# automl/TransformersCanDoBayesianInference

Hardware: AMD Instinct MI355X
Metric: synthetic datasets/sec (GP prior, bptt=2000) (higher is better)
Workload: dtype fp16; 1 GPU; priors.fast_gp, bptt=2000, num_features=18, emsize=512, nhead=4, nhid=1024, nlayers=6, 1000 bars (BASELINE.json configs[1]); per_gpu_batch=64, global_batch=64, aggregate_k_gradients=1, aggregate_streams=0, aggregate_stacked=False, seq_len=2000, parallelism=dp1, micro_batch_streams=2, eval_pos=weighted sampler(2000)

## Files before the change

include/pfn_hip.h:

```cpp
#ifndef PFN_HIP_H
#define PFN_HIP_H

#include <stddef.h>
#include <stdint.h>

#ifdef __cplusplus
extern "C" {
#endif

#define PFN_ABI_VERSION 10

enum {
  PFN_OK = 0,
  PFN_ERR_UNSUPPORTED = -1,
  PFN_ERR_ALIGNMENT = -2,
  PFN_ERR_LAUNCH = -3,
  PFN_ERR_ARGUMENT = -4,
};

enum { PFN_PREC_BF16 = 0,
       PFN_PREC_F32 = 1,
       PFN_PREC_FP16 = 2   };

typedef struct pfn_model_desc {
  int32_t num_features;
  int32_t emsize;
  int32_t nhead;
  int32_t nhid;
  int32_t nlayers;
  int32_t n_out;
  int32_t precision;
  float ln_eps;
  float dropout;
  int32_t schedule;
} pfn_model_desc;
enum { PFN_SCHED_TOP_LAYER_ALL_ROWS = 1,
       PFN_SCHED_FUSE_LN_WIDE = 2,
       PFN_SCHED_SEPARATE_LNBWD = 4,
       PFN_SCHED_NO_KEY_CENTERING = 16,
       PFN_SCHED_KEY_CENTERING = 64,
       PFN_SCHED_F32_RESIDUAL = 128,
       PFN_SCHED_FUSE_Q_PROJECTION = 32,
       PFN_SCHED_DETERMINISTIC = 8        };
int pfn_default_schedule(void);

int pfn_abi_version(void);
const char* pfn_last_error_string(void);
enum { PFN_TUNE_GEMM_NT_KERNEL = 0,
       PFN_TUNE_GEMM_TN_WRAP = 1,
       PFN_TUNE_FUSE_LNBWD = 2,
       PFN_TUNE_ATTN_PINGPONG = 4,
       PFN_TUNE_FUSE_LN_WIDE = 5,
       PFN_TUNE_GP_PLANES = 8,
       PFN_TUNE_FUSE_DELTA = 9,
       PFN_TUNE_GEMM_LN_ROWS = 7,
       PFN_TUNE_ATTN_BWD_GROUP = 10,
       PFN_TUNE_WGRAD_SPLITS = 11,
       PFN_TUNE_WGRAD_WAVES = 14,
       PFN_TUNE_LOSS_SCALE_TARGET = 15,
       PFN_TUNE_RESIDUAL16 = 16,
       PFN_TUNE_FUSE_Q_PROJECTION = 12,
       PFN_TUNE_KEY_CENTERING = 13,
       PFN_TUNE_ATTN_CACHE_SPLITS = 17,
       PFN_TUNE_TOP_LAYER_TEST_ROWS = 6  };
int pfn_set_tuning(int key, int value);
enum { PFN_PROF_ATTN_FWD = 0, PFN_PROF_ATTN_BWD_DELTA = 2, PFN_PROF_ATTN_BWD_KV = 4, PFN_PROF_ATTN_BWD_DQ = 6, PFN_PROF_GEMM_QKV = 8,
       PFN_PROF_GEMM_OUT_LN = 10, PFN_PROF_GEMM_LIN1 = 12, PFN_PROF_GEMM_LIN2_LN = 14, PFN_PROF_GEMM_DHPRE = 16, PFN_PROF_GEMM_DY1 = 18,
       PFN_PROF_GEMM_DCTX = 20, PFN_PROF_GEMM_DX = 22, PFN_PROF_WGRAD = 24, PFN_PROF_SLOTS = 26 };
int pfn_profile_enable(int on);
int pfn_profile_read(int slot, double* total_ms, int64_t* launches);

int pfn_param_layout(const pfn_model_desc* d, int64_t* offsets, int64_t* numels, int max_tensors);
int64_t pfn_param_count(const pfn_model_desc* d);
int64_t pfn_shadow_bytes(const pfn_model_desc* d);
int pfn_prepare_params(const pfn_model_desc* d, const float* params, void* shadow, void* stream);

int64_t pfn_workspace_bytes(const pfn_model_desc* d, int B, int S);
int64_t pfn_top_layer_rows(const pfn_model_desc* d, int B, int S, int sep, int use_dropout);
int pfn_stack_forward(const pfn_model_desc* d, const float* params, const void* shadow,
                      const float* x, int64_t x_st, int64_t x_sb,
                      const float* y, int64_t y_st, int64_t y_sb,
                      const float* src_sbe,
                      int B, int S, int sep,
                      void* workspace, int64_t workspace_bytes,
                      float* logits, void* stream);
int pfn_stack_forward_dropout(const pfn_model_desc* d, const float* params, const void* shadow,
                              const float* x, int64_t x_st, int64_t x_sb,
                              const float* y, int64_t y_st, int64_t y_sb,
                              const float* src_sbe,
                              int B, int S, int sep,
                              void* workspace, int64_t workspace_bytes,
                              float* logits, void* stream, uint64_t dropout_seed);
int pfn_stack_backward(const pfn_model_desc* d, const float* params, const void* shadow,
                       const float* x, int64_t x_st, int64_t x_sb,
                       const float* y, int64_t y_st, int64_t y_sb,
// ... 115 lines not shown
                     int B, int S, int nf, int kernel, float* nll, float* mean, float* var,
                     int32_t* info, void* stream);

int64_t pfn_gp_fit_workspace_bytes(int P, int S);
int pfn_gp_mll_grad(const float* x, const float* y, const int32_t* n_of, const float* theta, const float* prior,
                    int P, int S, int nf, int kernel, int flags, void* ws, int64_t ws_bytes,
                    float* value, float* grad, int32_t* info, void* stream);
int pfn_gp_fit_predict(const float* x, const float* y, const int32_t* n_of, const float* theta, const float* prior,
                       int P, int S, int nf, int kernel, const float* x_test, int m, void* ws, int64_t ws_bytes,
                       float* mean, float* var, int32_t* info, void* stream);

#define PFN_NUTS_ADAPT_MASS 1
#define PFN_NUTS_KEEP_WARMUP 2
#define PFN_NUTS_MAX_WINDOWS 16
#define PFN_NUTS_INV_MASS_OFFSET 256
int64_t pfn_nuts_workspace_bytes(int C, int D, int max_tree_depth);
int pfn_nuts_init(void* ws, int64_t ws_bytes, int C, int D, int64_t ld, int max_tree_depth, int num_warmup, int num_samples, int flags,
                  const int32_t* window_ends, int n_windows, int window_start, float step_size, float target_accept, uint64_t seed,
                  const int64_t* chain_ids, const float* theta0, const float* inv_mass0, float* trial, int32_t* done_count, void* stream);
int pfn_nuts_advance(void* ws, int64_t ws_bytes, int C, int D, int64_t ld, int max_tree_depth, int num_warmup, int num_samples,
                     const float* value, const float* grad, const int32_t* info, const float* scale, const float* shift, float* trial,
                     float* samples, float* stats, float* warm, int32_t* done_count, void* stream);

int pfn_bnn_logp_grad(const float* x, const float* y, const int32_t* n_of, const float* theta, int64_t ld,
                      int P, int K, int S, int F, int H, int activation,
                      float* value, float* grad, void* stream);
int pfn_bnn_predict(const float* x_test, const float* theta, int64_t ld, int P, int K, int m, int F, int H, int activation,
                    float* prob1, void* stream);

int pfn_bnn_svi_steps(const float* x, const float* y, const int32_t* n_of, float* state, int64_t ld, int P, int S, int F, int H, int activation,
                      int num_particles, int64_t step0, int num_steps, float lr, float beta1, float beta2, float eps, uint64_t seed,
                      const int64_t* problem_ids, float* loss, void* stream);

#define PFN_BNN_SVGD_MAX_PARTICLES 64
int64_t pfn_bnn_svgd_workspace_bytes(int P, int num_particles, int F, int H);
int pfn_bnn_svgd_steps(const float* x, const float* y, const int32_t* n_of, float* state, int64_t ld, int P, int S, int F, int H, int activation,
                       int num_particles, int64_t step0, int num_steps, float lr, float beta1, float beta2, float eps, float bandwidth_factor,
                       void* workspace, int64_t workspace_bytes, float* potential, float* bandwidth, void* stream);

int pfn_mlp_prior_forward(const float* weights, const float* biases, const int32_t* model_of, const int32_t* dims,
                          const float* noise_std, float* causes, const float* noise, float* y, float* hidden,
                          int B, int T, int HP, int Lmax, int activation, int gen_causes,
                          uint64_t seed, uint64_t offset, void* stream);

int pfn_op_gemm_nt(const void* A, int64_t lda, const void* B, int64_t ldb, int M, int N, int K,
                   int flags, const float* bias, const void* aux, int64_t ld_aux,
                   const float* resid, int64_t ld_resid, float* out_f32, int64_t ld_out_f32,
                   void* out_t, int64_t ld_out_t, void* out2_t, int64_t ld_out2, int prec, void* stream);
int pfn_op_gemm_tn(const void* A, int64_t lda, const void* B, int64_t ldb, float* C, int64_t ldc,
                   int M, int P, int Q, int atomic, int prec, void* stream);
int pfn_op_gemm_tn_group(int n, const void* const* A, const int64_t* lda, const void* const* B, const int64_t* ldb,
                         float* const* C, const int64_t* ldc, const int32_t* P, const int32_t* Q,
                         float* const* colsum, int M, int splits, int prec, void* stream);
#define PFN_OP_SUMS_16BIT 256
int pfn_op_gemm_ln(const void* A, int64_t lda, const void* B, int64_t ldb, int M, int N, int K, const float* bias,
                   const float* resid, const float* ry, const float* rmean, const float* rrstd,
                   const float* rgamma, const float* rbeta, const float* gamma, const float* beta, float eps,
                   float* y, float* mean, float* rstd, void* x_t, int prec, void* stream);
int pfn_op_gemm_lnbwd(const void* A, int64_t lda, const void* B, int64_t ldb, int M, int N, int K, const void* aux,
                      const float* y, const float* mean, const float* rstd, const float* gamma,
                      void* dx_t, float* dgamma, float* dbeta, int prec, void* stream);
int pfn_op_attention_fwd(const void* qkv, void* ctx, float* lse, int B, int S, int E, int H, int sep,
                         int prec, void* stream);
int64_t pfn_op_attention_bwd_ws_bytes(int B, int S, int H, int prec);
int pfn_op_attention_bwd(const void* qkv, const void* ctx, const float* lse, const void* dctx,
                         void* dqkv, float* delta_ws, void* ds_ws, int B, int S, int E, int H, int sep,
                         int prec, int parts, void* stream);
int pfn_op_attention_fwd_from(const void* qkv, void* ctx, float* lse, int B, int S, int E, int H, int sep, int q_begin,
                              int prec, void* stream);
int pfn_op_attention_bwd_from(const void* qkv, const void* ctx, const float* lse, const void* dctx,
                              void* dqkv, float* delta_ws, void* ds_ws, int B, int S, int E, int H, int sep, int q_begin,
                              int prec, int parts, void* stream);
int pfn_op_gather_rows(const void* src_bs, void* dst_tb, int B, int S, int64_t row_bytes, int sep, void* stream);
int pfn_op_scatter_rows(const void* src_tb, void* dst_bs, int B, int S, int64_t row_bytes, int sep, int zero_from, void* stream);
int pfn_op_layernorm_fwd(const float* x, const float* gamma, const float* beta, float* y_f32, void* y_t,
                         float* mean, float* rstd, int64_t rows, int E, float eps, int prec, void* stream);
int pfn_op_layernorm_bwd(const void* dy, int dy_is_t, const float* x, const float* gamma, const float* mean,
                         const float* rstd, float* dx_f32, void* dx_t, float* dgamma, float* dbeta,
                         float* dbias_extra, int64_t rows, int E, int prec, void* stream);
int pfn_op_cast(const float* src, void* dst, int64_t n, int prec, void* stream);
int pfn_op_qkv_projection(const void* x_t, const void* w_in_t, const float* b_in, void* qkv_t, float* kshift_ws,
                          int B, int S, int E, int sep, const int32_t* sep_of, int center, int prec, void* stream);

#ifdef __cplusplus
}
#endif
#endif
```

transformerscandobayesianinference_amd/_hip.py:

```python
import ctypes
import os
import subprocess

import torch

_HERE = os.path.dirname(os.path.abspath(__file__))
LIB_PATH = os.path.join(_HERE, 'libpfn_hip.so')
ABI_VERSION = 10

MAX_FEATURES = 1022
PREC_BF16 = 0
PREC_F32 = 1
PREC_FP16 = 2
PRECISIONS = {'bf16': PREC_BF16, 'f32': PREC_F32, 'fp32': PREC_F32, 'fp16': PREC_FP16, 'f16': PREC_FP16}
SCHED_TOP_LAYER_ALL_ROWS, SCHED_FUSE_LN_WIDE, SCHED_SEPARATE_LNBWD, SCHED_DETERMINISTIC, SCHED_NO_KEY_CENTERING, SCHED_FUSE_Q_PROJECTION, SCHED_KEY_CENTERING, SCHED_F32_RESIDUAL = 1, 2, 4, 8, 16, 32, 64, 128
NUTS_ADAPT_MASS, NUTS_KEEP_WARMUP, NUTS_MAX_WINDOWS, NUTS_INV_MASS_OFFSET = 1, 2, 16, 256

EPI_BIAS, EPI_GELU, EPI_GELU_BWD, EPI_RESID, EPI_OUT_F32, EPI_OUT_T, EPI_OUT2_T, EPI_ACCUM, EPI_RESID_T = 1, 2, 4, 8, 16, 32, 64, 128, 256


class HipExtensionError(RuntimeError):
    pass


class ModelDesc(ctypes.Structure):
    _fields_ = [('num_features', ctypes.c_int32), ('emsize', ctypes.c_int32), ('nhead', ctypes.c_int32),
                ('nhid', ctypes.c_int32), ('nlayers', ctypes.c_int32), ('n_out', ctypes.c_int32),
                ('precision', ctypes.c_int32), ('ln_eps', ctypes.c_float), ('dropout', ctypes.c_float), ('schedule', ctypes.c_int32)]

    def key(self):
        return (self.num_features, self.emsize, self.nhead, self.nhid, self.nlayers, self.n_out, self.precision, self.ln_eps, self.dropout, self.schedule)


HOST_CALLBACK = ctypes.CFUNCTYPE(None, ctypes.c_void_p)

_lib = None

_c = ctypes
_P, _I, _L, _F, _U64 = _c.c_void_p, _c.c_int, _c.c_int64, _c.c_float, _c.c_uint64
_D = _c.POINTER(ModelDesc)

SIGNATURES = {
    'pfn_abi_version': (_I, []),
    'pfn_last_error_string': (_c.c_char_p, []),
    'pfn_set_tuning': (_I, [_I, _I]),
    'pfn_default_schedule': (_I, []),
    'pfn_profile_enable': (_I, [_I]),
    'pfn_profile_read': (_I, [_I, _c.POINTER(_c.c_double), _c.POINTER(_L)]),
    'pfn_param_layout': (_I, [_D, _c.POINTER(_L), _c.POINTER(_L), _I]),
    'pfn_param_count': (_L, [_D]),
    'pfn_shadow_bytes': (_L, [_D]),
    'pfn_prepare_params': (_I, [_D, _P, _P, _P]),
    'pfn_workspace_bytes': (_L, [_D, _I, _I]),
    'pfn_top_layer_rows': (_L, [_D, _I, _I, _I, _I]),
    'pfn_stack_forward': (_I, [_D, _P, _P, _P, _L, _L, _P, _L, _L, _P, _I, _I, _I, _P, _L, _P, _P]),
    'pfn_stack_backward': (_I, [_D, _P, _P, _P, _L, _L, _P, _L, _L, _I, _I, _I, _P, _L, _P, _P, _P, _P]),
    'pfn_stack_forward_dropout': (_I, [_D, _P, _P, _P, _L, _L, _P, _L, _L, _P, _I, _I, _I, _P, _L, _P, _P, _U64]),
    'pfn_stack_backward_split': (_I, [_D, _P, _P, _P, _L, _L, _P, _L, _L, _I, _I, _I, _P, _L, _P, _P, _P, _P, _I, _P, _P, _I, _U64]),
    'pfn_stack_forward_ragged': (_I, [_D, _P, _P, _P, _L, _L, _P, _L, _L, _I, _I, _P, _P, _I, _I, _L, _P, _L, _P, _P, _I, _U64]),
    'pfn_stack_backward_ragged': (_I, [_D, _P, _P, _P, _L, _L, _P, _L, _L, _I, _I, _P, _P, _I, _I, _L, _P, _L, _P, _P, _P, _I, _P, _P, _I, _U64]),
    'pfn_context_bytes': (_L, [_D, _I, _I]),
    'pfn_stack_condition': (_I, [_D, _P, _P, _P, _L, _L, _P, _L, _L, _I, _I, _P, _L, _P, _L, _P]),
    'pfn_predict_workspace_bytes': (_L, [_D, _I, _I]),
    'pfn_stack_predict': (_I, [_D, _P, _P, _P, _L, _I, _P, _L, _L, _I, _I, _P, _L, _P, _P]),
    'pfn_predict_grad_workspace_bytes': (_L, [_D, _I, _I]),
    'pfn_stack_predict_saved': (_I, [_D, _P, _P, _P, _L, _I, _P, _L, _L, _I, _I, _P, _L, _P, _P]),
    'pfn_stack_predict_backward': (_I, [_D, _P, _P, _P, _L, _I, _I, _I, _P, _L, _P, _P, _L, _L, _P]),
    'pfn_stack_condition_ragged': (_I, [_D, _P, _P, _P, _L, _L, _P, _L, _L, _I, _I, _P, _P, _L, _P, _L, _P]),
    'pfn_stack_predict_ragged': (_I, [_D, _P, _P, _P, _L, _I, _P, _P, _L, _L, _I, _I, _P, _L, _P, _P]),
    'pfn_stack_predict_saved_ragged': (_I, [_D, _P, _P, _P, _L, _I, _P, _P, _L, _L, _I, _I, _P, _L, _P, _P]),
    'pfn_stack_predict_backward_ragged': (_I, [_D, _P, _P, _P, _L, _I, _P, _I, _I, _P, _L, _P, _P, _L, _L, _P]),
    'pfn_stack_input_grads': (_I, [_D, _P, _I, _I, _I, _P, _L, _P, _L, _L, _P, _L, _L, _P]),
    'pfn_bar_nll_forward': (_I, [_P, _L, _P, _P, _L, _I, _I, _P, _P, _P, _P]),
    'pfn_bar_nll_backward': (_I, [_P, _L, _P, _P, _P, _L, _I, _P, _P]),
    'pfn_bar_mean': (_I, [_P, _L, _P, _L, _I, _I, _P, _P]),
    'pfn_bar_mean_backward': (_I, [_P, _L, _P, _L, _I, _I, _P, _P, _P, _P]),
    'pfn_bar_stats': (_I, [_P, _L, _P, _L, _I, _I, _P, _I, _P, _L, _P, _P]),
    'pfn_bar_stats_backward': (_I, [_P, _L, _P, _L, _I, _I, _P, _I, _P, _L, _P, _P, _P, _P]),
    'pfn_bar_sample': (_I, [_P, _L, _P, _L, _I, _I, _I, _U64, _P, _P]),
    'pfn_clip_adam_step': (_I, [_P, _P, _P, _P, _L, _F, _F, _F, _F, _F, _F, _I, _I, _P, _P]),
    'pfn_gp_workspace_bytes': (_L, [_I, _I]),
    'pfn_gp_prior_sample': (_I, [_P, _P, _P, _P, _L, _P, _P, _P, _I, _I, _I, _I, _I, _I, _U64, _U64, _P, _P]),
    'pfn_gp_posterior': (_I, [_P, _P, _P, _L, _P, _P, _P, _P, _P, _I, _I, _I, _I, _P, _P, _P, _P, _P]),
    'pfn_gp_fit_workspace_bytes': (_L, [_I, _I]),
    'pfn_gp_mll_grad': (_I, [_P, _P, _P, _P, _P, _I, _I, _I, _I, _I, _P, _L, _P, _P, _P, _P]),
    'pfn_gp_fit_predict': (_I, [_P, _P, _P, _P, _P, _I, _I, _I, _I, _P, _I, _P, _L, _P, _P, _P, _P]),
    'pfn_nuts_workspace_bytes': (_L, [_I, _I, _I]),
    'pfn_nuts_init': (_I, [_P, _L, _I, _I, _L, _I, _I, _I, _I, _P, _I, _I, _F, _F, _U64, _P, _P, _P, _P, _P, _P]),
    'pfn_nuts_advance': (_I, [_P, _L, _I, _I, _L, _I, _I, _I, _P, _P, _P, _P, _P, _P, _P, _P, _P, _P, _P]),
    'pfn_bnn_logp_grad': (_I, [_P, _P, _P, _P, _L, _I, _I, _I, _I, _I, _I, _P, _P, _P]),
    'pfn_bnn_predict': (_I, [_P, _P, _L, _I, _I, _I, _I, _I, _I, _P, _P]),
    'pfn_bnn_svi_steps': (_I, [_P, _P, _P, _P, _L, _I, _I, _I, _I, _I, _I, _L, _I, _F, _F, _F, _F, _U64, _P, _P, _P]),
    'pfn_bnn_svgd_workspace_bytes': (_L, [_I, _I, _I, _I]),
    'pfn_bnn_svgd_steps': (_I, [_P, _P, _P, _P, _L, _I, _I, _I, _I, _I, _I, _L, _I, _F, _F, _F, _F, _F, _P, _L, _P, _P, _P]),
    'pfn_mlp_prior_forward': (_I, [_P, _P, _P, _P, _P, _P, _P, _P, _P, _I, _I, _I, _I, _I, _I, _U64, _U64, _P]),
    'pfn_op_gemm_nt': (_I, [_P, _L, _P, _L, _I, _I, _I, _I, _P, _P, _L, _P, _L, _P, _L, _P, _L, _P, _L, _I, _P]),
    'pfn_op_gemm_tn': (_I, [_P, _L, _P, _L, _P, _L, _I, _I, _I, _I, _I, _P]),
    'pfn_op_gemm_tn_group': (_I, [_I, _P, _P, _P, _P, _P, _P, _P, _P, _P, _I, _I, _I, _P]),
    'pfn_op_gemm_ln': (_I, [_P, _L, _P, _L, _I, _I, _I, _P, _P, _P, _P, _P, _P, _P, _P, _P, _F, _P, _P, _P, _P, _I, _P]),
    'pfn_op_gemm_lnbwd': (_I, [_P, _L, _P, _L, _I, _I, _I, _P, _P, _P, _P, _P, _P, _P, _P, _I, _P]),
    'pfn_op_attention_fwd': (_I, [_P, _P, _P, _I, _I, _I, _I, _I, _I, _P]),
    'pfn_op_attention_bwd_ws_bytes': (_L, [_I, _I, _I, _I]),
    'pfn_op_attention_fwd_from': (_I, [_P, _P, _P, _I, _I, _I, _I, _I, _I, _I, _P]),
    'pfn_op_attention_bwd_from': (_I, [_P, _P, _P, _P, _P, _P, _P, _I, _I, _I, _I, _I, _I, _I, _I, _P]),
    'pfn_op_gather_rows': (_I, [_P, _P, _I, _I, _L, _I, _P]),
    'pfn_op_scatter_rows': (_I, [_P, _P, _I, _I, _L, _I, _I, _P]),
    'pfn_op_attention_bwd': (_I, [_P, _P, _P, _P, _P, _P, _P, _I, _I, _I, _I, _I, _I, _I, _P]),
    'pfn_op_layernorm_fwd': (_I, [_P, _P, _P, _P, _P, _P, _P, _L, _I, _F, _I, _P]),
    'pfn_op_layernorm_bwd': (_I, [_P, _I, _P, _P, _P, _P, _P, _P, _P, _P, _P, _L, _I, _I, _P]),
    'pfn_op_cast': (_I, [_P, _P, _L, _I, _P]),
    'pfn_op_qkv_projection': (_I, [_P, _P, _P, _P, _P, _I, _I, _I, _I, _P, _I, _I, _P]),
}


def build(verbose=False):
    script = os.path.join(_HERE, 'csrc', 'build.sh')
    res = subprocess.run(['bash', script], capture_output=True, text=True)
    if res.returncode != 0 or not os.path.exists(LIB_PATH):
        raise HipExtensionError('building libpfn_hip.so failed:\n' + res.stdout[-4000:] + res.stderr[-8000:])
    if verbose:
        print(res.stdout[-2000:])
    return LIB_PATH


def lib():
    global _lib
    if _lib is None:
        if not os.path.exists(LIB_PATH):
            raise HipExtensionError(
                f'{LIB_PATH} not found. Build it with `python -c "import __graft_entry__ as g; g.build()"` '
                f'(or transformerscandobayesianinference_amd/csrc/build.sh). There is no CPU / PyTorch fallback for the hot path.')
        handle = ctypes.CDLL(LIB_PATH)
        for name, (res, args) in SIGNATURES.items():
            try:
                fn = getattr(handle, name)
            except AttributeError as e:
                raise HipExtensionError(f'libpfn_hip.so does not export {name}') from e
            fn.restype = res
            fn.argtypes = args
        if handle.pfn_abi_version() != ABI_VERSION:
            raise HipExtensionError(f'libpfn_hip.so ABI {handle.pfn_abi_version()} != binding ABI {ABI_VERSION}; rebuild')
        _lib = handle
    return _lib


def check(rc, what):
    if rc < 0:
        msg = lib().pfn_last_error_string()
        raise HipExtensionError(f'{what} failed with code {rc}: {msg.decode() if msg else ""}')
    return rc

# ... 15 lines not shown
```

transformerscandobayesianinference_amd/csrc/gemm_tn.hip:

```cpp
#include <type_traits>
#include "pfn_device.h"
#include "pfn_kernels.h"

namespace pfn {

PFN_DEV int xcd_remap(int bid, int nwg) {
  const int q = nwg >> 3, r = nwg & 7, xcd = bid & 7;
  return (xcd < r ? xcd * (q + 1) : r * (q + 1) + (xcd - r) * q) + (bid >> 3);
}
typedef __attribute__((address_space(1))) const void gvoid_t;
typedef __attribute__((address_space(3))) void lvoid_t;

constexpr int TN_BMK = 32;

template <typename T>
__global__ __launch_bounds__(256, 2) void gemm_tn_kernel(GemmTN g) {
  constexpr int RB = 128 * sizeof(T);
  constexpr int TILE = TN_BMK * RB;
  extern __shared__ __attribute__((aligned(16))) char smem_raw[];
  LdsPtr smem = lds_cast(smem_raw);
  auto tileA = [&](int buf) { return smem + buf * 2 * TILE; };
  auto tileB = [&](int buf) { return smem + buf * 2 * TILE + TILE; };

  const int p0 = blockIdx.y * 128, q0 = blockIdx.x * 128;
  const int colsA = min(128, g.P - p0), colsB = min(128, g.Q - q0);
  const long mbeg = (long)blockIdx.z * g.m_chunk;
  const long mend = min((long)g.M, mbeg + g.m_chunk);
  if (mbeg >= mend) return;
  const T* A = reinterpret_cast<const T*>(g.A) + mbeg * g.lda + p0;
  const T* B = reinterpret_cast<const T*>(g.B) + mbeg * g.ldb + q0;

  const int wave = threadIdx.x >> 6, lane = threadIdx.x & 63;
  const int wp = wave >> 1, wq = wave & 1;

  f32x16 acc[2][2];
#pragma unroll
  for (int i = 0; i < 2; ++i)
#pragma unroll
    for (int j = 0; j < 2; ++j)
#pragma unroll
      for (int r = 0; r < 16; ++r) acc[i][j][r] = 0.f;

  TileStage<T, TN_BMK, RB, 256> sa, sb;
  const int rows_total = (int)(mend - mbeg);
  const int nt = (rows_total + TN_BMK - 1) / TN_BMK;
  const bool do_colsum = g.colsum != nullptr && blockIdx.x == 0;
  constexpr int EPC = 16 / sizeof(T);
  float csum[EPC];
#pragma unroll
  for (int e = 0; e < EPC; ++e) csum[e] = 0.f;
  auto add_colsum = [&]() {
    if (!do_colsum) return;
// ... 81 lines not shown
#ifndef PFN_TNB_KT
#define PFN_TNB_KT 64
#define PFN_TNB_NS 2
#endif
#ifndef PFN_TNB_LATE_ISSUE
#define PFN_TNB_LATE_ISSUE 1
#endif
constexpr int TNB_KT = PFN_TNB_KT;
constexpr int TNB_NS = PFN_TNB_NS;
constexpr int TNB_TILE = TNB_KT * 512;
constexpr int TNB_PW = TNB_KT / 16;
constexpr int TNB_LDS = TNB_NS * 2 * TNB_TILE;
static_assert(TNB_LDS <= 160 * 1024 && TNB_KT % 16 == 0 && TNB_NS >= 2 && (TNB_NS - 2) * 2 * TNB_PW < 64, "weight-gradient ring does not fit");
constexpr long TN_GROUP_MAX_SPLIT_BYTES = 0x7ffffff0L;

template <int NW> struct TnStager {
  static constexpr int NP = TNB_KT / 2 / NW;
  DmaRsrc ra, rb;
  unsigned a_lo, a_hi, b_lo, b_hi;
  unsigned step_a, step_b;
  int va[NP], vb[NP];
  int wave, srow, mask;
  PFN_DEV void init(const TnProblem& pr, long mbeg, int rows, int p0, int q0, int wave_, int lane, int debug_mask) {
    const long lda2 = pr.lda * 2, ldb2 = pr.ldb * 2;
    ra = make_dma_rsrc(reinterpret_cast<const char*>(pr.A) + mbeg * lda2 + p0 * 2, (rows - 1) * lda2 + 512);
    rb = make_dma_rsrc(reinterpret_cast<const char*>(pr.B) + mbeg * ldb2 + q0 * 2, (rows - 1) * ldb2 + 512);
    a_lo = ra.w[0]; a_hi = ra.w[1]; b_lo = rb.w[0]; b_hi = rb.w[1];
    step_a = __builtin_amdgcn_readfirstlane((unsigned)(TNB_KT * lda2));
    step_b = __builtin_amdgcn_readfirstlane((unsigned)(TNB_KT * ldb2));
    wave = wave_; srow = 0; mask = debug_mask;
    const int row0 = wave * 2 + (lane >> 5);
    const int colb = ((((lane & 31) >> 2) ^ (row0 & 3)) * 32 + (lane & 3) * 8) * 2;
#pragma unroll
    for (int i = 0; i < NP; ++i) {
      va[i] = (row0 + 2 * NW * i) * (int)lda2 + colb;
      vb[i] = (row0 + 2 * NW * i) * (int)ldb2 + colb;
    }
  }
  PFN_DEV void issue(LdsPtr slot) {
    LdsPtr ta = slot + wave * 1024;
    LdsPtr tb = ta + TNB_TILE;
#pragma unroll
    for (int i = 0; i < NP; ++i) {
      dma16(ra, ta + i * NW * 1024, va[i]);
      dma16(rb, tb + i * NW * 1024, vb[i]);
    }
    dma_rsrc_advance(ra, step_a);
    dma_rsrc_advance(rb, step_b);
    srow += TNB_KT;
    if ((srow & mask) == 0) { ra.w[0] = a_lo; ra.w[1] = a_hi; rb.w[0] = b_lo; rb.w[1] = b_hi; }
  }
};

template <typename T>
__global__ __launch_bounds__(512, 1) void gemm_tn_big_kernel(GemmTNGroup g) {
  extern __shared__ __attribute__((aligned(16))) char smem_raw[];
  LdsPtr smem = lds_cast(smem_raw);

  const int ntiles = g.tile_start[g.n];
  const int id = xcd_remap(blockIdx.x, ntiles * g.splits);
  const int split = id / ntiles, tile = id % ntiles;
  int pi = 0;
  while (tile >= g.tile_start[pi + 1]) ++pi;
  const TnProblem& pr = g.p[pi];
  const int tq = pr.Q / 256;
  const int tl = tile - g.tile_start[pi];
  const int p0 = (tl / tq) * 256, q0 = (tl % tq) * 256;
  const long mbeg = (long)split * g.m_chunk;
  const long mend = min((long)g.M, mbeg + g.m_chunk);
  const int rows_total = (int)(mend - mbeg);
  if (rows_total <= 0) return;

  const int wave = __builtin_amdgcn_readfirstlane(threadIdx.x >> 6), lane = threadIdx.x & 63;
  const int wp = wave >> 2, wq = wave & 3;

  TnStager<8> stg;
  stg.init(pr, mbeg, rows_total, p0, q0, wave, lane, g.debug_mask);
  static_assert(TnStager<8>::NP == TNB_PW, "wait_stage counts 2 TNB_PW DMA instructions per stage");

  f32x16 acc[4][2];
#pragma unroll
  for (int i = 0; i < 4; ++i)
#pragma unroll
    for (int j = 0; j < 2; ++j)
#pragma unroll
      for (int r = 0; r < 16; ++r) acc[i][j][r] = 0.f;
  f32x16 cs;
#pragma unroll
  for (int r = 0; r < 16; ++r) cs[r] = 0.f;
  const bool do_colsum = pr.colsum != nullptr && q0 == 0;
  Frag<T> ones;
#pragma unroll
  for (int e = 0; e < 8; ++e) ones.v[e] = (T)1.0f;

  const int nt = (rows_total + TNB_KT - 1) / TNB_KT;
#pragma unroll
  for (int st = 0; st < TNB_NS - 1; ++st)
    if (st < nt) stg.issue(smem + st * 2 * TNB_TILE);
  auto wait_stage = [&](int younger) {
    if constexpr (TNB_NS == 2) { wait_vm_barrier<0>(); return; }
    switch (younger) {
      case 0: wait_vm_barrier<0>(); break;
      case 1: wait_vm_barrier<(TNB_NS > 2 ? 1 : 0) * 2 * TNB_PW>(); break;
      case 2: wait_vm_barrier<(TNB_NS > 3 ? 2 : 0) * 2 * TNB_PW>(); break;
      case 3: wait_vm_barrier<(TNB_NS > 4 ? 3 : 0) * 2 * TNB_PW>(); break;
      default: wait_vm_barrier<(TNB_NS - 2) * 2 * TNB_PW>(); break;
    }
  };
  static_assert(TNB_NS <= 6, "wait_stage cases");
  auto main_loop = [&](auto with_colsum) {
    constexpr bool CS = decltype(with_colsum)::value;
    int slot = 0, slot_next = TNB_NS - 1;
    for (int t = 0; t < nt; ++t) {
      wait_stage(min(nt - t - 1, TNB_NS - 2));
      const bool more = t + TNB_NS - 1 < nt;
      if (!PFN_TNB_LATE_ISSUE && more) stg.issue(smem + slot_next * 2 * TNB_TILE);
      LdsPtr ta = smem + slot * 2 * TNB_TILE;
      LdsPtr tb = ta + TNB_TILE;
#pragma unroll
      for (int ks = 0; ks < TNB_KT; ks += 16) {
        Frag<T> fa[4], fb[2];
#pragma unroll
        for (int j = 0; j < 2; ++j) fb[j] = load_frag_tr<T, 512, 1>(tb, ks, wq * 64 + j * 32);
#pragma unroll
        for (int i = 0; i < 4; ++i) fa[i] = load_frag_tr<T, 512, 1>(ta, ks, wp * 128 + i * 32);
#pragma unroll
        for (int i = 0; i < 4; ++i)
#pragma unroll
          for (int j = 0; j < 2; ++j) acc[i][j] = mma32(fa[i], fb[j], acc[i][j]);
        if constexpr (CS) cs = mma32(load_frag_tr<T, 512, 1>(ta, ks, wp * 128 + wq * 32), ones, cs);
        if (PFN_TNB_LATE_ISSUE && ks == 0) {
          PFN_PIN_LDS_MFMA();
          if (more) stg.issue(smem + slot_next * 2 * TNB_TILE);
          PFN_PIN_LDS_MFMA();
        }
      }
      slot_next = slot;
      slot = slot + 1 == TNB_NS ? 0 : slot + 1;
    }
  };
  if (do_colsum) main_loop(std::true_type{});
  else main_loop(std::false_type{});

  const int pv = pr.Pv > 0 ? pr.Pv : pr.P;
  const float osc = loss_scale_down(g.scale_amax);
  if (do_colsum && (lane & 31) == 0) {
#pragma unroll
    for (int r = 0; r < 16; ++r) {
      const int pp = p0 + wp * 128 + wq * 32 + acc_row(r, lane);
      if (pp < pv) unsafeAtomicAdd(pr.colsum + pp, cs[r] * osc);
    }
  }
  const bool atomic = true;
#pragma unroll
  for (int i = 0; i < 4; ++i)
#pragma unroll
    for (int j = 0; j < 2; ++j)
#pragma unroll
      for (int r = 0; r < 16; ++r) {
        const int pp = p0 + wp * 128 + i * 32 + acc_row(r, lane);
        const int qq = q0 + wq * 64 + j * 32 + (lane & 31);
        float* c = pr.C + (long)pp * pr.ldc + qq;
        if (pp >= pv) continue;
        if (atomic) unsafeAtomicAdd(c, acc[i][j][r] * osc);
        else *c += acc[i][j][r] * osc;
      }
}

#define PFN_TNW_BUILT (PFN_TNB_KT == 64 && PFN_TNB_NS == 2)
#if PFN_TNW_BUILT
constexpr int TNW_NW = 4;
template <typename T>
__global__ __launch_bounds__(TNW_NW * 64, 1) void gemm_tn_wide_kernel(GemmTNGroup g) {
  extern __shared__ __attribute__((aligned(16))) char smem_raw[];
  LdsPtr smem = lds_cast(smem_raw);
  const int ntiles = g.tile_start[g.n];
  const int id = xcd_remap(blockIdx.x, ntiles * g.splits);
  const int split = id / ntiles, tile = id % ntiles;
  int pi = 0;
  while (tile >= g.tile_start[pi + 1]) ++pi;
  const TnProblem& pr = g.p[pi];
  const int tq = pr.Q / 256;
  const int tl = tile - g.tile_start[pi];
  const int p0 = (tl / tq) * 256, q0 = (tl % tq) * 256;
  const long mbeg = (long)split * g.m_chunk;
  const long mend = min((long)g.M, mbeg + g.m_chunk);
  const int rows_total = (int)(mend - mbeg);
  if (rows_total <= 0) return;
  const int wave = __builtin_amdgcn_readfirstlane(threadIdx.x >> 6), lane = threadIdx.x & 63;
  const int wp = wave >> 1, wq = wave & 1;

  TnStager<TNW_NW> stg;
  stg.init(pr, mbeg, rows_total, p0, q0, wave, lane, g.debug_mask);

  f32x16 acc[4][4];
#pragma unroll
  for (int i = 0; i < 4; ++i)
#pragma unroll
    for (int j = 0; j < 4; ++j)
#pragma unroll
      for (int r = 0; r < 16; ++r) acc[i][j][r] = 0.f;
  float cs[2] = {0.f, 0.f};
  const bool do_colsum = pr.colsum != nullptr && q0 == 0;

  const int nt = (rows_total + TNB_KT - 1) / TNB_KT;
  struct Frs { Frag<T> a[4], b[4]; };
  auto main_loop = [&](auto with_colsum) {
    constexpr bool CS = decltype(with_colsum)::value;
    Frs f0, f1;
    auto ld = [&](Frs& f, const lds_char* ta, const lds_char* tb, int ks) {
#pragma unroll
      for (int j = 0; j < 4; ++j) f.b[j] = load_frag_tr<T, 512, 1>(tb, ks, wq * 128 + j * 32);
#pragma unroll
      for (int i = 0; i < 4; ++i) f.a[i] = load_frag_tr<T, 512, 1>(ta, ks, wp * 128 + i * 32);
    };
    auto mm = [&](const Frs& f) {
#pragma unroll
      for (int i = 0; i < 4; ++i)
#pragma unroll
        for (int j = 0; j < 4; ++j) acc[i][j] = mma32(f.a[i], f.b[j], acc[i][j]);
      if constexpr (CS) {
#pragma unroll
        for (int c = 0; c < 2; ++c)
#pragma unroll
          for (int e = 0; e < 8; ++e) cs[c] += (float)(wq ? f.a[2 + c] : f.a[c]).v[e];
      }
    };
    auto enter_stage = [&](int t, int slot) {
      wait_vm_barrier<0>();
      if (t + 1 < nt) stg.issue(smem + (slot ^ 1) * 2 * TNB_TILE);
    };
    int slot = 0;
    enter_stage(0, slot);
    ld(f0, smem, smem + TNB_TILE, 0);
    for (int t = 0; t < nt; ++t) {
      const lds_char* ta = smem + slot * 2 * TNB_TILE;
      const lds_char* tb = ta + TNB_TILE;
      ld(f1, ta, tb, 16);
      PFN_PIN_LDS_MFMA();
      mm(f0);
// ... 27 lines not shown
#pragma unroll
    for (int c = 0; c < 2; ++c) {
      const float s = cs[c] + __shfl_xor(cs[c], 32, 64);
      const int pp = p0 + wp * 128 + (2 * wq + c) * 32 + (lane & 31);
      if (lane < 32 && pp < pv) unsafeAtomicAdd(pr.colsum + pp, s * osc);
    }
  }
#pragma unroll
  for (int i = 0; i < 4; ++i)
#pragma unroll
    for (int j = 0; j < 4; ++j)
#pragma unroll
      for (int r = 0; r < 16; ++r) {
        const int pp = p0 + wp * 128 + i * 32 + acc_row(r, lane);
        const int qq = q0 + wq * 128 + j * 32 + (lane & 31);
        if (pp < pv) unsafeAtomicAdd(pr.C + (long)pp * pr.ldc + qq, acc[i][j][r] * osc);
      }
}
#endif

static bool aligned16(const void* p) { return (reinterpret_cast<uintptr_t>(p) & 15) == 0; }

static int g_tn_debug_wrap = 0;
void set_gemm_tn_debug_wrap(int rows) { g_tn_debug_wrap = rows; }
static int g_tn_group_splits = 0;
void set_gemm_tn_group_splits(int splits) { g_tn_group_splits = splits; }
static bool g_tn_wide = false;
void set_gemm_tn_group_waves(int waves) { g_tn_wide = waves == 4; }

int launch_gemm_tn(GemmTN g, int precision, hipStream_t stream) {
  if (g.M <= 0 || g.P <= 0 || g.Q <= 0) return PFN_OK;
  const size_t es = prec_esize(precision);
  if ((g.lda * es) % 16 || (g.ldb * es) % 16 || !aligned16(g.A) || !aligned16(g.B)) return PFN_ERR_ALIGNMENT;
  const int tp = (g.P + 127) / 128, tq = (g.Q + 127) / 128;
  int splits = (1024 + tp * tq - 1) / (tp * tq);
  const int max_splits = (g.M + 4 * TN_BMK - 1) / (4 * TN_BMK);
  if (splits > max_splits) splits = max_splits;
  if (g.max_splits > 0 && splits > g.max_splits) splits = g.max_splits;
  if (splits < 1) splits = 1;
  if (!g.atomic) splits = 1;
  int chunk = (g.M + splits - 1) / splits;
  chunk = (chunk + TN_BMK - 1) / TN_BMK * TN_BMK;
  splits = (g.M + chunk - 1) / chunk;
  g.m_chunk = chunk;
  const size_t lds = 4 * TN_BMK * 128 * es;
  PFN_DISPATCH_OP(precision, hipLaunchKernelGGL(gemm_tn_kernel<T>, dim3(tq, tp, splits), dim3(256), lds, stream, g));
  return hipGetLastError() == hipSuccess ? PFN_OK : PFN_ERR_LAUNCH;
}

bool gemm_tn_group_supported(const TnProblem& p) {
  return p.P % 256 == 0 && p.Q % 256 == 0 && (p.lda * 2) % 16 == 0 && (p.ldb * 2) % 16 == 0 && aligned16(p.A) && aligned16(p.B);
}

int launch_gemm_tn_group(GemmTNGroup g, int precision, hipStream_t stream) {
  if (g.n <= 0 || g.M <= 0) return PFN_OK;
  if (g.n > TN_GROUP_MAX) return PFN_ERR_ARGUMENT;
  if (!prec_is16(precision)) return PFN_ERR_UNSUPPORTED;
  int tiles = 0;
  for (int i = 0; i < g.n; ++i) {
    if (!gemm_tn_group_supported(g.p[i])) return PFN_ERR_UNSUPPORTED;
    g.tile_start[i] = tiles;
    tiles += (g.p[i].P / 256) * (g.p[i].Q / 256);
  }
  g.tile_start[g.n] = tiles;
  int splits = g.splits;
  if (splits <= 0 && g_tn_group_splits > 0) splits = g_tn_group_splits;
  if (splits <= 0) {
    splits = 8;
    for (int sp = 1; sp <= 8; ++sp) {
      const int blocks = tiles * sp, rounds = (blocks + 255) / 256;
      if (blocks >= 0.9 * rounds * 256) { splits = sp; break; }
    }
  }
  const int max_splits = (g.M + 4 * TNB_KT - 1) / (4 * TNB_KT);
  if (splits > max_splits) splits = max_splits;
  int chunk = (g.M + splits - 1) / splits;
  chunk = (chunk + TNB_KT - 1) / TNB_KT * TNB_KT;
  splits = (g.M + chunk - 1) / chunk;
  g.splits = splits;
  g.m_chunk = chunk;
  for (int i = 0; i < g.n; ++i) {
    const TnProblem& p = g.p[i];
    if (p.lda < 256 || p.ldb < 256 || (long)chunk * p.lda * 2 > TN_GROUP_MAX_SPLIT_BYTES || (long)chunk * p.ldb * 2 > TN_GROUP_MAX_SPLIT_BYTES) return PFN_ERR_UNSUPPORTED;
  }
  const int wrap = g_tn_debug_wrap;
  g.debug_mask = wrap >= TNB_KT && (wrap & (wrap - 1)) == 0 ? wrap - 1 : 0x7fffffff;
  if (g_tn_wide) {
#if PFN_TNW_BUILT
    static LdsAllowance allow_w[2];
    if (precision == PFN_PREC_FP16) {
      allow_w[1].ensure(gemm_tn_wide_kernel<f16>, TNB_LDS);
      hipLaunchKernelGGL(gemm_tn_wide_kernel<f16>, dim3(tiles * splits), dim3(TNW_NW * 64), TNB_LDS, stream, g);
    } else {
      allow_w[0].ensure(gemm_tn_wide_kernel<bf16>, TNB_LDS);
      hipLaunchKernelGGL(gemm_tn_wide_kernel<bf16>, dim3(tiles * splits), dim3(TNW_NW * 64), TNB_LDS, stream, g);
    }
    return hipGetLastError() == hipSuccess ? PFN_OK : PFN_ERR_LAUNCH;
#else
    return PFN_ERR_UNSUPPORTED;
#endif
  }
  static LdsAllowance allowance[2];
  if (precision == PFN_PREC_FP16) {
    allowance[1].ensure(gemm_tn_big_kernel<f16>, TNB_LDS);
    hipLaunchKernelGGL(gemm_tn_big_kernel<f16>, dim3(tiles * splits), dim3(512), TNB_LDS, stream, g);
  } else {
    allowance[0].ensure(gemm_tn_big_kernel<bf16>, TNB_LDS);
    hipLaunchKernelGGL(gemm_tn_big_kernel<bf16>, dim3(tiles * splits), dim3(512), TNB_LDS, stream, g);
  }
  return hipGetLastError() == hipSuccess ? PFN_OK : PFN_ERR_LAUNCH;
}

}
```

transformerscandobayesianinference_amd/csrc/pfn_api.hip:

```cpp
#include <algorithm>
#include <cstdarg>
#include <cstdio>
#include <cstring>
#include <mutex>
#include <vector>
#include "pfn_kernels.h"

using namespace pfn;

namespace pfn {
namespace {
struct ProfPair { hipEvent_t a, b; };
std::mutex g_prof_mu;
std::vector<ProfPair> g_prof[PFN_PROF_SLOTS];
std::atomic<int> g_prof_on{0};
}
bool prof_enabled() { return g_prof_on.load(std::memory_order_relaxed) != 0; }
void* prof_begin(int slot, hipStream_t s) {
  const int on = g_prof_on.load(std::memory_order_relaxed);
  if (!on || slot < 0 || slot >= PFN_PROF_SLOTS) return nullptr;
  if (on >= 2 && (slot & ~1) != on - 2) return nullptr;
  ProfPair* p = new ProfPair;
  if (hipEventCreate(&p->a) != hipSuccess || hipEventCreate(&p->b) != hipSuccess) { delete p; return nullptr; }
  (void)hipEventRecord(p->a, s);
  return p;
}
void prof_end(void* token, int slot, hipStream_t s) {
  if (!token) return;
  ProfPair* p = (ProfPair*)token;
  (void)hipEventRecord(p->b, s);
  std::lock_guard<std::mutex> lock(g_prof_mu);
  g_prof[slot].push_back(*p);
  delete p;
}
}

namespace {

thread_local char g_err[512] = "";
int fail(int code, const char* fmt, ...) __attribute__((format(printf, 2, 3)));
int fail(int code, const char* fmt, ...) {
  va_list ap;
  va_start(ap, fmt);
  vsnprintf(g_err, sizeof(g_err), fmt, ap);
  va_end(ap);
  return code;
}
#define PFN_TRY(expr)                                                                   \
  do {                                                                                  \
    int rc_ = (expr);                                                                   \
    if (rc_ != PFN_OK) return fail(rc_, "%s failed with %d at %s:%d", #expr, rc_, __FILE__, __LINE__); \
  } while (0)

inline int64_t align_up(int64_t v, int64_t a) { return (v + a - 1) / a * a; }
inline int esize(int prec) { return prec_esize(prec); }

int check_desc(const pfn_model_desc* d) {
  if (!d) return fail(PFN_ERR_ARGUMENT, "null model descriptor");
  if (d->precision != PFN_PREC_BF16 && d->precision != PFN_PREC_F32 && d->precision != PFN_PREC_FP16) return fail(PFN_ERR_ARGUMENT, "bad precision %d", d->precision);
  if (d->num_features < 1 || d->emsize < 8 || d->nhead < 1 || d->nhid < 8 || d->nlayers < 0 || d->n_out < 0)
    return fail(PFN_ERR_ARGUMENT, "bad model dimensions");
  if (d->num_features > EMB_MAX_FEATURES) return fail(PFN_ERR_UNSUPPORTED, "num_features %d > %d unsupported (the embedding stages 16 tokens x (num_features + 2) f32 in 64 KB of LDS)", d->num_features, EMB_MAX_FEATURES);
  if (d->emsize % d->nhead) return fail(PFN_ERR_ARGUMENT, "emsize %d not divisible by nhead %d", d->emsize, d->nhead);
  if (d->emsize % 8 || d->nhid % 8) return fail(PFN_ERR_UNSUPPORTED, "emsize and nhid must be multiples of 8 (16-byte operand rows)");
  const int dh = d->emsize / d->nhead;
  const bool ok = dh == 32 || dh == 64 || dh == 128 || dh == 256;
  if (!ok) return fail(PFN_ERR_UNSUPPORTED, "head dim %d unsupported (32/64/128/256)", dh);
  if (d->emsize > 2048) return fail(PFN_ERR_UNSUPPORTED, "emsize > 2048 unsupported by the LayerNorm kernels");
  if (d->schedule & ~(PFN_SCHED_TOP_LAYER_ALL_ROWS | PFN_SCHED_FUSE_LN_WIDE | PFN_SCHED_SEPARATE_LNBWD | PFN_SCHED_DETERMINISTIC | PFN_SCHED_NO_KEY_CENTERING | PFN_SCHED_FUSE_Q_PROJECTION | PFN_SCHED_KEY_CENTERING | PFN_SCHED_F32_RESIDUAL)) return fail(PFN_ERR_ARGUMENT, "unknown schedule bits 0x%x", d->schedule);
  if (!(d->dropout >= 0.f && d->dropout < 1.f)) return fail(PFN_ERR_ARGUMENT, "dropout %g outside [0, 1)", (double)d->dropout);
  return PFN_OK;
}

struct LayerP { int64_t w_in, b_in, w_o, b_o, w1, b1, w2, b2, g1, be1, g2, be2; };
struct Layout {
  int64_t enc_w, enc_b, yenc_w, yenc_b;
  std::vector<LayerP> layer;
  int64_t dec0_w, dec0_b, dec2_w, dec2_b;
  int64_t total;
  std::vector<LayerP> layer_t;
  int64_t dec0_wt, dec2_wt, total_t;
  int n_out_pad;
  std::vector<int64_t> offsets, numels;
};

Layout make_layout(const pfn_model_desc& d) {
  Layout L;
  const int64_t E = d.emsize, F = d.nhid, nf = d.num_features, O = d.n_out;
  int64_t cur = 0;
  auto take = [&](int64_t n) { int64_t o = cur; L.offsets.push_back(o); L.numels.push_back(n); cur = align_up(cur + n, 64); return o; };
  L.enc_w = take(E * nf); L.enc_b = take(E); L.yenc_w = take(E); L.yenc_b = take(E);
  L.layer.resize(d.nlayers);
  for (auto& p : L.layer) {
    p.w_in = take(3 * E * E); p.b_in = take(3 * E); p.w_o = take(E * E); p.b_o = take(E);
    p.w1 = take(F * E); p.b1 = take(F); p.w2 = take(E * F); p.b2 = take(E);
    p.g1 = take(E); p.be1 = take(E); p.g2 = take(E); p.be2 = take(E);
  }
  if (O > 0) { L.dec0_w = take(F * E); L.dec0_b = take(F); L.dec2_w = take(O * F); L.dec2_b = take(O); }
  else L.dec0_w = L.dec0_b = L.dec2_w = L.dec2_b = 0;
  L.total = cur;
  L.n_out_pad = (int)align_up(O, O >= 64 ? 64 : 8);
  int64_t ct = 0;
  auto take_t = [&](int64_t n) { int64_t o = ct; ct = align_up(ct + n, 64); return o; };
  L.layer_t.resize(d.nlayers);
  for (auto& p : L.layer_t) { p.w_in = take_t(3 * E * E); p.w_o = take_t(E * E); p.w1 = take_t(F * E); p.w2 = take_t(E * F); }
  if (O > 0) { L.dec0_wt = take_t(F * E); L.dec2_wt = take_t(F * (int64_t)L.n_out_pad); }
  else L.dec0_wt = L.dec2_wt = 0;
  L.total_t = ct;
  return L;
}

struct LayerWs {
  char *qkv, *ctx, *x1_t, *hpre, *h, *x2_t; float *lse, *y1, *mean1, *rstd1, *x1, *y2, *mean2, *rstd2, *x2;
  char *dy2_t, *dh_t, *dy1_t, *dqkv_t;
  char *dy2m_t, *dy1m_t;
};
struct Ws {
  float* x0; char* x0_t;
  char* xaug_t;
  float* embacc;
  float* xaug_amax;
  std::vector<LayerWs> layer;
  char *xt_t, *dpre, *dt;
  char *dlog_t, *dd_t, *dctx_t;
  float *dxt, *gA, *delta;
  char* ds;
  char* gA_t;
  char *top_ctx_t, *top_dy1_t, *top_dctx_t;
  float *top_ry, *top_rmean, *top_rrstd;
  float* kshift;
  float* lscale;
  float* ln_part;
  int64_t bytes;
};

struct Ragged { const int32_t* sep_of; const int64_t* row_off; int64_t test_rows; int sep_min; };

static bool key_centering(const pfn_model_desc& d) {
  return (d.precision == PFN_PREC_FP16 && !(d.schedule & PFN_SCHED_NO_KEY_CENTERING)) || (d.precision == PFN_PREC_BF16 && (d.schedule & PFN_SCHED_KEY_CENTERING));
}

static bool residual16(const pfn_model_desc& d) {
  const int E = d.emsize;
  const bool wide = (d.schedule & PFN_SCHED_FUSE_LN_WIDE) != 0;
  return d.precision == PFN_PREC_FP16 && !(d.schedule & PFN_SCHED_F32_RESIDUAL) && d.nlayers > 0 && d.dropout == 0.f && d.nhid % 32 == 0 &&
         (E == 128 || E == 256 || E == 512 || (E == 1024 && wide));
}
static bool residual16_separate_ln(const pfn_model_desc& d, bool ln_fusable) {
  return d.precision == PFN_PREC_FP16 && !(d.schedule & PFN_SCHED_F32_RESIDUAL) && d.nlayers > 0 && d.dropout == 0.f && d.emsize >= 1024 && d.emsize % 8 == 0 && !ln_fusable;
}

Ws carve(const pfn_model_desc& d, int B, int S, char* base) {
  Ws w;
  const int64_t M = (int64_t)B * S, E = d.emsize, F = d.nhid, es = esize(d.precision);
  const int64_t npad = align_up(d.n_out, 8);
  int64_t cur = 0;
  auto take = [&](int64_t nbytes) { char* p = base ? base + cur : nullptr; cur = align_up(cur + nbytes, 256); return p; };
  w.x0 = (float*)take(M * E * 4); w.x0_t = take(M * E * es);
  const int64_t aug = emb_aug_width(d.num_features) > 0 ? emb_aug_width(d.num_features) : 32;
  w.xaug_t = take(M * aug * es); w.embacc = (float*)take(E * aug * 4);
  w.xaug_amax = (float*)take(aug * 4);
  w.layer.resize(d.nlayers);
  for (auto& l : w.layer) {
    l.qkv = take(M * 3 * E * es); l.ctx = take(M * E * es); l.lse = (float*)take((int64_t)B * d.nhead * S * 4);
    l.y1 = (float*)take(M * E * 4); l.mean1 = (float*)take(M * 4); l.rstd1 = (float*)take(M * 4);
    l.x1 = (float*)take(M * E * 4); l.x1_t = take(M * E * es);
    l.hpre = take(M * F * es); l.h = take(M * F * es);
    l.y2 = (float*)take(M * E * 4); l.mean2 = (float*)take(M * 4); l.rstd2 = (float*)take(M * 4);
    l.x2 = (float*)take(M * E * 4); l.x2_t = take(M * E * es);
    l.dy2_t = take(M * E * es); l.dh_t = take(M * F * es); l.dy1_t = take(M * E * es); l.dqkv_t = take(M * 3 * E * es);
    l.dy2m_t = l.dy1m_t = nullptr;
    if (d.dropout > 0.f) { l.dy2m_t = take(M * E * es); l.dy1m_t = take(M * E * es); }
  }
  w.xt_t = take(M * E * es); w.dpre = take(M * F * es); w.dt = take(M * F * es);
  w.dlog_t = take(M * npad * es); w.dd_t = take(M * F * es); w.dxt = (float*)take(M * E * 4);
  w.gA = (float*)take(M * E * 4); w.gA_t = take(M * E * es);
  w.dctx_t = take(M * E * es);
  w.delta = (float*)take(2 * (int64_t)B * d.nhead * S * 4);
  w.ds = take(attn_bwd_ds_bytes(B, S, d.nhead, d.precision));
  const int64_t Mtop = (d.nlayers > 0 && d.dropout == 0.f && !(d.schedule & PFN_SCHED_TOP_LAYER_ALL_ROWS)) ? (int64_t)B * (S - (S + 3) / 4) : 0;
  w.top_ctx_t = take(Mtop * E * es); w.top_dy1_t = take(Mtop * E * es); w.top_dctx_t = take(Mtop * E * es);
  w.top_ry = (float*)take(Mtop * E * 4); w.top_rmean = (float*)take(Mtop * 4); w.top_rrstd = (float*)take(Mtop * 4);
  w.kshift = key_centering(d) ? (float*)take((int64_t)B * E * 4) : nullptr;
  w.lscale = (float*)take(256);
  w.ln_part = (d.schedule & PFN_SCHED_DETERMINISTIC) ? (float*)take((int64_t)LNB_MAX_BLOCKS * 3 * E * 4) : nullptr;
  w.bytes = cur;
  return w;
}

struct Context { int64_t kv_bytes, shift_bytes, layer_bytes, bytes; };
static bool context_centred(const pfn_model_desc& d) { return key_centering(d) && d.emsize % 64 == 0; }
Context context_layout(const pfn_model_desc& d, int B, int sep) {
  Context c;
  c.kv_bytes = align_up((int64_t)B * sep * 2 * d.emsize * esize(d.precision), 256);
  c.shift_bytes = context_centred(d) ? align_up((int64_t)B * d.emsize * 4, 256) : 0;
  c.layer_bytes = sep > 0 ? c.kv_bytes + c.shift_bytes : 0;
  c.bytes = c.layer_bytes * d.nlayers;
  return c;
}
struct KvSink { char* base; Context c; };

struct PredictWs {
  float *x2, *y2, *mean2, *rstd2; char* x2_t;
  float *x1, *y1, *mean1, *rstd1; char* x1_t;
  char *qkv, *ctx, *h, *hpre;
  float *part_o, *part_ml;
  int64_t bytes;
};
PredictWs carve_predict(const pfn_model_desc& d, int B, int n, char* base) {
  PredictWs w;
  const int64_t M = (int64_t)B * n, E = d.emsize, F = d.nhid, es = esize(d.precision);
  const int64_t nsplit = attn_cache_splits(B, n, d.emsize, d.nhead, -1, d.precision);
  int64_t cur = 0;
  auto take = [&](int64_t nbytes) { char* p = base ? base + cur : nullptr; cur = align_up(cur + nbytes, 256); return p; };
// ... 50 lines not shown
  return g;
}
GemmTN tn(const void* A, long lda, const void* B, long ldb, float* C, long ldc, int M, int P, int Q, float* colsum = nullptr) {
  GemmTN g;
  memset(&g, 0, sizeof(g));
  g.A = A; g.lda = lda; g.B = B; g.ldb = ldb; g.C = C; g.ldc = ldc; g.M = M; g.P = P; g.Q = Q; g.atomic = 1; g.colsum = colsum;
  return g;
}

struct Model { const pfn_model_desc* d; const float* params; const char* sh; const Layout* L; hipStream_t s; };
inline const void* W(const Model& m, int64_t off) { return m.sh + off * esize(m.d->precision); }
inline const void* WT(const Model& m, int64_t off) { return m.sh + (m.L->total + off) * esize(m.d->precision); }
constexpr int NO_PROF = -PFN_PROF_SLOTS;

int check_context(const pfn_model_desc& d, int B, int sep, const void* context, int64_t context_bytes, Context* c) {
  *c = context_layout(d, B, sep);
  if (sep > 0 && d.nlayers > 0 && !context) return fail(PFN_ERR_ARGUMENT, "null context with sep=%d", sep);
  if (context_bytes < c->bytes) return fail(PFN_ERR_ARGUMENT, "context too small: %lld < %lld", (long long)context_bytes, (long long)c->bytes);
  return PFN_OK;
}

bool ln_gemm_probe(const pfn_model_desc& d, float* x0, void* x0_t, const float* params, const void* sh, int M) {
  GemmLN probe; memset(&probe, 0, sizeof(probe));
  probe.A = x0_t; probe.lda = d.emsize; probe.B = sh; probe.ldb = d.emsize; probe.M = M; probe.N = d.emsize; probe.K = d.emsize;
  probe.bias = params; probe.gamma = params; probe.beta = params; probe.resid = x0; probe.y = x0; probe.x_t = x0_t;
  return gemm_ln_supported(probe);
}

struct Plan {
  bool ln_ok;
  bool fuse_ln;
  bool y16;
  bool y16u;
  bool y16_any;
  bool lnb_eligible;
};
Plan make_plan(const pfn_model_desc& d, float* x0, void* x0_t, const float* params, const void* sh, int M, float pdrop) {
  Plan pl;
  const int E = d.emsize, sched = d.schedule;
  const bool width_ok = (E <= 512 || (sched & PFN_SCHED_FUSE_LN_WIDE));
  pl.ln_ok = ln_gemm_probe(d, x0, x0_t, params, sh, M);
  const bool ln_fusable = pl.ln_ok && d.nhid % 32 == 0 && width_ok;
  pl.fuse_ln = prec_is16(d.precision) && ln_fusable && pdrop == 0.f;
  pl.y16 = residual16(d) && pl.ln_ok;
  pl.y16u = residual16_separate_ln(d, ln_fusable);
  pl.y16_any = pl.y16 || pl.y16u;
  pl.lnb_eligible = !(sched & PFN_SCHED_DETERMINISTIC) && !(sched & PFN_SCHED_SEPARATE_LNBWD) && prec_is16(d.precision) && d.nlayers > 0 && pdrop == 0.f && width_ok;
  return pl;
}

bool emb_gemm(const pfn_model_desc& d, bool custom_encoder) {
  return !custom_encoder && prec_is16(d.precision) && d.nlayers > 0 && emb_aug_width(d.num_features) > 0 && d.emsize % 8 == 0;
}
bool predict_dsrc_is_t(const pfn_model_desc& d) { return d.nlayers > 0 && prec_is16(d.precision); }

struct Resid { const float* plain; const void* y; const float* mean; const float* rstd; const float* gamma; const float* beta; };
void set_resid(GemmLN& g, const Resid& r) { g.resid = r.plain; g.ry = r.y; g.rmean = r.mean; g.rrstd = r.rstd; g.rgamma = r.gamma; g.rbeta = r.beta; }
struct LayerBufs { const float* xin; const char* xin_t; char *qkv, *ctx; float* lse; float *y1, *mean1, *rstd1, *x1; char *x1_t, *h, *hpre; float *y2, *mean2, *rstd2, *x2; char* x2_t; };

int layer_tail_forward(const Model& m, const LayerP& p, const LayerBufs& u, Resid& res, int rows, const Plan& pl, float pdrop, const unsigned* seed, bool last, int prof) {
  const pfn_model_desc& d = *m.d;
  const int prec = d.precision, E = d.emsize, F = d.nhid;
  const float* params = m.params;
  hipStream_t s = m.s;
  const bool y16u = pl.y16u;
  if (pl.fuse_ln) {
    ProfScope ps(PFN_PROF_GEMM_OUT_LN + prof, s);
    GemmLN g; memset(&g, 0, sizeof(g));
    g.A = u.ctx; g.lda = E; g.B = W(m, p.w_o); g.ldb = E; g.M = rows; g.N = E; g.K = E; g.bias = params + p.b_o;
    set_resid(g, res);
    g.gamma = params + p.g1; g.beta = params + p.be1; g.eps = d.ln_eps;
    g.y = u.y1; g.mean = u.mean1; g.rstd = u.rstd1; g.x_t = u.x1_t; g.y16 = pl.y16;
    PFN_TRY(launch_gemm_ln(g, prec, s));
    res = Resid{nullptr, u.y1, u.mean1, u.rstd1, params + p.g1, params + p.be1};
  } else {
    {
      GemmNT g = nt(u.ctx, E, W(m, p.w_o), E, rows, E, E, EPI_BIAS | (pdrop > 0.f ? 0 : EPI_RESID) | EPI_OUT_F32);
      g.bias = params + p.b_o; g.resid = u.xin; g.ld_resid = E; g.out_f32 = u.y1; g.ld_out_f32 = E;
      if (y16u) { g.flags = EPI_BIAS | EPI_RESID_T | EPI_OUT_T; g.aux = u.xin_t; g.ld_aux = E; g.out_t = u.y1; g.ld_out_t = E; }
      PFN_TRY(launch_gemm_nt(g, prec, s));
      if (pdrop > 0.f) PFN_TRY(launch_dropout_add(u.y1, u.xin, rows, E, seed[1], pdrop, s));
    }
    PFN_TRY(launch_layernorm_fwd(u.y1, params + p.g1, params + p.be1, y16u ? nullptr : u.x1, u.x1_t, u.mean1, u.rstd1, rows, E, d.ln_eps, prec, s, y16u));
  }
  {
    ProfScope ps(PFN_PROF_GEMM_LIN1 + prof, s);
    GemmNT g = nt(u.x1_t, E, W(m, p.w1), E, rows, F, E, EPI_BIAS | EPI_GELU | EPI_OUT_T | EPI_OUT2_T);
    g.bias = params + p.b1; g.out_t = u.h; g.ld_out_t = F; g.out2_t = u.hpre; g.ld_out2 = F;
    PFN_TRY(launch_gemm_nt(g, prec, s));
    if (pdrop > 0.f) PFN_TRY(launch_dropout_scale(u.h, u.h, u.hpre, u.hpre, rows, F, seed[2], pdrop, prec, s));
  }
  if (pl.fuse_ln) {
    ProfScope ps(PFN_PROF_GEMM_LIN2_LN + prof, s);
    GemmLN g; memset(&g, 0, sizeof(g));
    g.A = u.h; g.lda = F; g.B = W(m, p.w2); g.ldb = F; g.M = rows; g.N = E; g.K = F; g.bias = params + p.b2;
    set_resid(g, res);
    g.gamma = params + p.g2; g.beta = params + p.be2; g.eps = d.ln_eps;
    g.y = u.y2; g.mean = u.mean2; g.rstd = u.rstd2; g.x_t = u.x2_t; g.y16 = pl.y16;
    g.x_f32 = last ? u.x2 : nullptr;
    PFN_TRY(launch_gemm_ln(g, prec, s));
    res = Resid{nullptr, u.y2, u.mean2, u.rstd2, params + p.g2, params + p.be2};
  } else {
    {
      GemmNT g = nt(u.h, F, W(m, p.w2), F, rows, E, F, EPI_BIAS | (pdrop > 0.f ? 0 : EPI_RESID) | EPI_OUT_F32);
      g.bias = params + p.b2; g.resid = u.x1; g.ld_resid = E; g.out_f32 = u.y2; g.ld_out_f32 = E;
      if (y16u) { g.flags = EPI_BIAS | EPI_RESID_T | EPI_OUT_T; g.aux = u.x1_t; g.ld_aux = E; g.out_t = u.y2; g.ld_out_t = E; }
      PFN_TRY(launch_gemm_nt(g, prec, s));
      if (pdrop > 0.f) PFN_TRY(launch_dropout_add(u.y2, u.x1, rows, E, seed[3], pdrop, s));
    }
    PFN_TRY(launch_layernorm_fwd(u.y2, params + p.g2, params + p.be2, (y16u && !last) ? nullptr : u.x2, u.x2_t, u.mean2, u.rstd2, rows, E, d.ln_eps, prec, s, y16u));
  }
  return PFN_OK;
}

int decoder_forward(const Model& m, const void* xt_t, char* dt, char* dpre, float* logits, int rows) {
  const int prec = m.d->precision, E = m.d->emsize, F = m.d->nhid, O = m.d->n_out;
  {
    GemmNT g = nt(xt_t, E, W(m, m.L->dec0_w), E, rows, F, E, EPI_BIAS | EPI_GELU | EPI_OUT_T | EPI_OUT2_T);
    g.bias = m.params + m.L->dec0_b; g.out_t = dt; g.ld_out_t = F; g.out2_t = dpre; g.ld_out2 = F;
    PFN_TRY(launch_gemm_nt(g, prec, m.s));
  }
  GemmNT g = nt(dt, F, W(m, m.L->dec2_w), F, rows, O, F, EPI_BIAS | EPI_OUT_F32);
  g.bias = m.params + m.L->dec2_b; g.out_f32 = logits; g.ld_out_f32 = O;
  return launch_gemm_nt(g, prec, m.s);
}
int decoder_backward_data(const Model& m, const void* dlog_t, const void* dpre, char* dd_t, float* dxt, int rows) {
  const int prec = m.d->precision, E = m.d->emsize, F = m.d->nhid, O = m.d->n_out, npad = m.L->n_out_pad;
  {
    GemmNT g = nt(dlog_t, npad, WT(m, m.L->dec2_wt), npad, rows, F, npad % 64 == 0 ? npad : O, EPI_GELU_BWD | EPI_OUT_T);
    g.aux = dpre; g.ld_aux = F; g.out_t = dd_t; g.ld_out_t = F;
    PFN_TRY(launch_gemm_nt(g, prec, m.s));
  }
  GemmNT g = nt(dd_t, F, WT(m, m.L->dec0_wt), F, rows, E, F, EPI_OUT_F32);
  g.out_f32 = dxt; g.ld_out_f32 = E;
  return launch_gemm_nt(g, prec, m.s);
}

bool tn_set_groupable(const std::vector<TnProblem>& probs, int prec) {
  bool grouped = prec_is16(prec);
  for (const TnProblem& t : probs) grouped = grouped && gemm_tn_group_supported(t);
  return grouped;
}
int launch_tn_set(const std::vector<TnProblem>& probs, int rows, int prec, bool det, const float* lsc, int prof_slot, hipStream_t s, bool allow_group = true) {
  auto one_by_one = [&](size_t i0, size_t n) {
    for (size_t i = i0; i < i0 + n; ++i) {
      const TnProblem& t = probs[i];
      GemmTN g = tn(t.A, t.lda, t.B, t.ldb, t.C, t.ldc, rows, t.Pv ? t.Pv : t.P, t.Q, t.colsum);
      if (det) g.max_splits = 1;
      g.scale_amax = lsc;
      PFN_TRY(launch_gemm_tn(g, prec, s));
    }
    return (int)PFN_OK;
  };
  if (!(allow_group && tn_set_groupable(probs, prec))) return one_by_one(0, probs.size());
  for (size_t i0 = 0; i0 < probs.size(); i0 += TN_GROUP_MAX) {
    ProfScope ps(prof_slot, s);
    GemmTNGroup g;
    memset(&g, 0, sizeof(g));
    g.n = (int)std::min<size_t>(TN_GROUP_MAX, probs.size() - i0);
    g.M = rows;
    g.splits = det ? 1 : 0;
    g.scale_amax = lsc;
    for (int i = 0; i < g.n; ++i) g.p[i] = probs[i0 + i];
    const int rc = launch_gemm_tn_group(g, prec, s);
    if (rc == PFN_ERR_UNSUPPORTED) PFN_TRY(one_by_one(i0, g.n));
    else PFN_TRY(rc);
  }
  return PFN_OK;
}

struct LnSinks { float *dgamma, *dbeta, *dbias; };
struct LayerGrads {
  const void* dout; int dout_is_t;
  const void* y2; const float *mean2, *rstd2, *gamma2; const void* y1; const float *mean1, *rstd1, *gamma1; const void* hpre;
  char *dy2_t, *dy2m_t, *dh_t, *dy1_t, *dqkv_t, *dx1_t;
  LnSinks ln2, ln1;
  float* ln_part;
};
GemmLNB lnb(const Model& m, const Plan& pl, const float* lsc, const void* A, long lda, const void* Bw, long ldb, int K, const void* aux, const void* y,
            const float* mean, const float* rstd, const float* gamma, void* dx_t, const LnSinks& sink, int rows) {
  GemmLNB g; memset(&g, 0, sizeof(g));
  g.A = A; g.lda = lda; g.B = Bw; g.ldb = ldb; g.M = rows; g.N = m.d->emsize; g.K = K; g.aux = aux;
  g.y = y; g.mean = mean; g.rstd = rstd; g.gamma = gamma; g.dx_t = dx_t; g.dgamma = sink.dgamma; g.dbeta = sink.dbeta; g.scale_amax = lsc; g.y16 = pl.y16_any;
  return g;
}
GemmLNB lnb_dy1(const Model& m, const Plan& pl, const float* lsc, const LayerP& t, const LayerGrads& g, int rows) {
  const int F = m.d->nhid;
  return lnb(m, pl, lsc, g.dh_t, F, WT(m, t.w1), F, F, g.dy2_t, g.y1, g.mean1, g.rstd1, g.gamma1, g.dy1_t, g.ln1, rows);
}
GemmLNB lnb_dx(const Model& m, const Plan& pl, const float* lsc, const LayerP& t, const char* dqkv_t, const char* dy1_t, const LayerGrads& below, int rows) {
  const int E = m.d->emsize;
  return lnb(m, pl, lsc, dqkv_t, 3 * E, WT(m, t.w_in), 3 * E, 3 * E, dy1_t, below.y2, below.mean2, below.rstd2, below.gamma2, below.dy2_t, below.ln2, rows);
}
bool lnbwd_fusable(const Model& m, const Plan& pl, const float* lsc, const LayerGrads& g0, int rows) {
  const LayerP& t = m.L->layer_t[0];
  return pl.lnb_eligible && gemm_lnbwd_supported(lnb_dy1(m, pl, lsc, t, g0, rows)) && gemm_lnbwd_supported(lnb_dx(m, pl, lsc, t, g0.dqkv_t, g0.dy1_t, g0, rows));
}
int layer_backward_to_dy1(const Model& m, const LayerP& t, const LayerGrads& g, int rows, const Plan& pl, bool fuse_lnb, bool ln2_done, const float* lsc,
                          float pdrop, unsigned seed2, int prof) {
  const int prec = m.d->precision, E = m.d->emsize, F = m.d->nhid;
// ... 155 lines not shown
  if (d->n_out > 0) {
    PFN_TRY(add(L.dec0_w, L.dec0_wt, F, E, F));
    PFN_TRY(add(L.dec2_w, L.dec2_wt, d->n_out, F, L.n_out_pad));
  }
  return launch_transpose_cast_group(params, tr, g, prec, s);
}

static int stack_forward_impl(const pfn_model_desc* d, const float* params, const void* shadow,
                              const float* x, int64_t x_st, int64_t x_sb, const float* y, int64_t y_st, int64_t y_sb,
                              const float* src_sbe, int B, int S, int sep, void* workspace, int64_t workspace_bytes,
                              float* logits, void* stream, bool use_dropout, uint64_t dropout_seed, const Ragged* rg = nullptr, const KvSink* sink = nullptr);
int pfn_stack_forward(const pfn_model_desc* d, const float* params, const void* shadow,
                      const float* x, int64_t x_st, int64_t x_sb, const float* y, int64_t y_st, int64_t y_sb,
                      const float* src_sbe, int B, int S, int sep, void* workspace, int64_t workspace_bytes,
                      float* logits, void* stream) {
  return stack_forward_impl(d, params, shadow, x, x_st, x_sb, y, y_st, y_sb, src_sbe, B, S, sep, workspace, workspace_bytes, logits, stream, false, 0);
}
int pfn_stack_forward_dropout(const pfn_model_desc* d, const float* params, const void* shadow,
                              const float* x, int64_t x_st, int64_t x_sb, const float* y, int64_t y_st, int64_t y_sb,
                              const float* src_sbe, int B, int S, int sep, void* workspace, int64_t workspace_bytes,
                              float* logits, void* stream, uint64_t dropout_seed) {
  return stack_forward_impl(d, params, shadow, x, x_st, x_sb, y, y_st, y_sb, src_sbe, B, S, sep, workspace, workspace_bytes, logits, stream, true, dropout_seed);
}
static int stack_forward_impl(const pfn_model_desc* d, const float* params, const void* shadow,
                              const float* x, int64_t x_st, int64_t x_sb, const float* y, int64_t y_st, int64_t y_sb,
                              const float* src_sbe, int B, int S, int sep, void* workspace, int64_t workspace_bytes,
                              float* logits, void* stream, bool use_dropout, uint64_t dropout_seed, const Ragged* rg, const KvSink* sink) {
  PFN_TRY(check_desc(d));
  const float pdrop = use_dropout ? d->dropout : 0.f;
  auto dseed = [&](int layer, int site) { return dropout_site_seed(dropout_seed, layer, site); };
  if (!params || !shadow || !workspace) return fail(PFN_ERR_ARGUMENT, "null pointer");
  if (!src_sbe && (!x || !y)) return fail(PFN_ERR_ARGUMENT, "need x and y (or src_sbe)");
  if (B < 1 || S < 1 || sep < 0 || sep > S) return fail(PFN_ERR_ARGUMENT, "bad B=%d S=%d sep=%d", B, S, sep);
  if (!logits && sep < S) return fail(PFN_ERR_ARGUMENT, "null logits");
  hipStream_t s = (hipStream_t)stream;
  const int prec = d->precision, es = esize(prec);
  const int E = d->emsize, H = d->nhead, O = d->n_out;
  Layout L = make_layout(*d);
  Ws w = carve(*d, B, S, (char*)workspace);
  if (workspace_bytes < w.bytes) return fail(PFN_ERR_ARGUMENT, "workspace too small: %lld < %lld", (long long)workspace_bytes, (long long)w.bytes);
  const int* sep_of = rg ? rg->sep_of : nullptr;
  if (rg && (src_sbe || rg->test_rows < 0 || rg->test_rows > (int64_t)B * S || !rg->sep_of || (!rg->row_off && !(sink && rg->test_rows == 0))))
    return fail(PFN_ERR_ARGUMENT, "bad ragged-batch arguments");
  const int M = B * S, Mt = rg ? (int)rg->test_rows : (S - sep) * B;
  const char* sh = (const char*)shadow;

  if (src_sbe) {
    PFN_TRY(launch_sbe_to_bse(src_sbe, w.x0, w.x0_t, S, B, E, prec, s));
  } else {
    EmbedArgs e;
    e.x = x; e.x_st = x_st; e.x_sb = x_sb; e.y = y; e.y_st = y_st; e.y_sb = y_sb;
    e.wx = params + L.enc_w; e.bx = params + L.enc_b; e.wy = params + L.yenc_w; e.by = params + L.yenc_b;
    e.out_f32 = w.x0; e.out_t = w.x0_t; e.S = S; e.B = B; e.nf = d->num_features; e.E = E; e.sep = sep; e.sep_of = sep_of;
    e.xaug_ld = emb_aug_width(d->num_features);
    e.xaug_t = e.xaug_ld > 0 ? w.xaug_t : nullptr;
    e.xaug_amax = nullptr;
    if (e.xaug_t && prec == PFN_PREC_FP16) {
      PFN_TRY(launch_embed_colmax(e, w.xaug_amax, s));
      e.xaug_amax = w.xaug_amax;
    }
    PFN_TRY(launch_embed_fwd(e, prec, s));
  }
  const float* xin = w.x0;
  const char* xin_t = w.x0_t;
  const Model m = {d, params, sh, &L, s};
  const Plan pl = make_plan(*d, w.x0, w.x0_t, params, sh, M, pdrop);
  Resid res = {w.x0, nullptr, nullptr, nullptr, nullptr, nullptr};
  const bool top_mode = rg ? top_layer_on_test_rows_ragged(*d, S, *rg, pdrop) : top_layer_on_test_rows(*d, S, sep, pdrop);
  const bool fuse_q = (d->schedule & PFN_SCHED_FUSE_Q_PROJECTION) && pdrop == 0.f && attn_fwd_can_fuse_q(E, H, prec);
  auto gather_top = [&](const void* src, void* dst, long row_bytes) {
    return rg ? launch_gather_rows_ragged(src, dst, S, B, row_bytes, rg->sep_of, (const long*)rg->row_off, s) : launch_gather_rows(src, dst, S, B, row_bytes, sep, s);
  };
  for (int l = 0; l < d->nlayers; ++l) {
    const LayerP& p = L.layer[l];
    LayerWs& a = w.layer[l];
    const bool top = top_mode && l == d->nlayers - 1;
    const int Ml = top ? Mt : M;
    {
      ProfScope ps(PFN_PROF_GEMM_QKV, s);
      GemmNT g = nt(xin_t, E, W(m, p.w_in), E, M, 3 * E, E, EPI_BIAS | EPI_OUT_T);
      g.bias = params + p.b_in; g.out_t = a.qkv; g.ld_out_t = 3 * E;
      if (fuse_q) {
        g.B = W(m, p.w_in + (int64_t)E * E); g.N = 2 * E; g.bias = params + p.b_in + E; g.out_t = a.qkv + (int64_t)E * es;
      }
      if (w.kshift && E % 64 == 0) {
        PFN_TRY(launch_key_shift(xin_t, W(m, p.w_in + (int64_t)E * E), w.kshift, B, S, E, sep, sep_of, prec, s));
        g.flags |= EPI_ROWSHIFT; g.rowshift = w.kshift; g.rs_ld = E; g.rs_S = S; g.rs_n0 = fuse_q ? 0 : E; g.rs_n1 = g.rs_n0 + E;
      }
      PFN_TRY(launch_gemm_nt(g, prec, s));
    }
    if (sink) {
      char* kv = sink->base + l * sink->c.layer_bytes;
      if (hipMemcpy2DAsync(kv, 2 * E * es, a.qkv + (int64_t)E * es, 3 * E * es, 2 * E * es, (size_t)M, hipMemcpyDeviceToDevice, s) != hipSuccess)
        return fail(PFN_ERR_LAUNCH, "context copy of layer %d", l);
      if (sink->c.shift_bytes && hipMemcpyAsync(kv + sink->c.kv_bytes, w.kshift, (size_t)B * E * 4, hipMemcpyDeviceToDevice, s) != hipSuccess)
        return fail(PFN_ERR_LAUNCH, "key shift copy of layer %d", l);
      if (l == d->nlayers - 1) break;
    }
    {
      AttnArgs at; memset(&at, 0, sizeof(at));
      at.qkv = a.qkv; at.ctx = a.ctx; at.lse = a.lse; at.B = B; at.S = S; at.E = E; at.H = H; at.sep = sep; at.sep_of = sep_of;
      at.p_drop = pdrop; at.drop_seed = dseed(l, 0);
      at.q_begin = top ? (rg ? rg->sep_min : sep) : 0;
      at.q_from_sep = (top && rg) ? 1 : 0;
      if (fuse_q) { at.xq = xin_t; at.wq = W(m, p.w_in); at.bq = params + p.b_in; at.q_store = 1; }
      PFN_TRY(launch_attn_fwd(at, prec, s));
    }
// ... 301 lines not shown
  if (!params || !shadow || !workspace || !grads) return fail(PFN_ERR_ARGUMENT, "null pointer");
  if (!dsrc_sbe && (!x || !y)) return fail(PFN_ERR_ARGUMENT, "need x and y (or dsrc_sbe)");
  if (B < 1 || S < 1 || sep < 0 || sep > S) return fail(PFN_ERR_ARGUMENT, "bad B=%d S=%d sep=%d", B, S, sep);
  hipStream_t s = (hipStream_t)stream;
  const int prec = d->precision, es = esize(prec);
  const int E = d->emsize, F = d->nhid, H = d->nhead, O = d->n_out;
  Layout L = make_layout(*d);
  Ws w = carve(*d, B, S, (char*)workspace);
  if (workspace_bytes < w.bytes) return fail(PFN_ERR_ARGUMENT, "workspace too small");
  const int M = B * S, Mt = rg ? (int)rg->test_rows : (S - sep) * B, npad = L.n_out_pad;
  const char* sh = (const char*)shadow;
  const Model m = {d, params, sh, &L, s};
  const Plan pl = make_plan(*d, w.x0, w.x0_t, params, sh, M, pdrop);

  if (prec == PFN_PREC_FP16 && Mt > 0) {
    if (!dlogits) return fail(PFN_ERR_ARGUMENT, "null dlogits");
    PFN_TRY(launch_absmax(dlogits, (long)Mt * (O > 0 ? O : E), w.lscale, s));
    lsc = w.lscale;
  }
  const float* dxt = w.dxt;
  const char* xt_t = top_mode ? w.layer[d->nlayers - 1].x2_t : w.xt_t;
  if (Mt > 0 && O == 0) {
    if (!dlogits) return fail(PFN_ERR_ARGUMENT, "null dlogits");
    dxt = dlogits;
    if (lsc) { PFN_TRY(launch_scale_copy(dlogits, w.dxt, (long)Mt * E, lsc, s)); dxt = w.dxt; }
  } else if (Mt > 0) {
    if (!dlogits) return fail(PFN_ERR_ARGUMENT, "null dlogits");
    PFN_TRY(launch_cast_rows(dlogits, O, w.dlog_t, npad, Mt, O, prec, s, lsc));
    TnProblem dp2; memset(&dp2, 0, sizeof(dp2));
    dp2.A = w.dlog_t; dp2.lda = npad; dp2.B = w.dt; dp2.ldb = F; dp2.C = grads + L.dec2_w; dp2.ldc = F; dp2.P = npad; dp2.Q = F; dp2.Pv = O;
    dp2.colsum = grads + L.dec2_b;
    TnProblem dp0; memset(&dp0, 0, sizeof(dp0));
    dp0.A = w.dd_t; dp0.lda = F; dp0.B = xt_t; dp0.ldb = E; dp0.C = grads + L.dec0_w; dp0.ldc = E; dp0.P = F; dp0.Q = E; dp0.colsum = grads + L.dec0_b;
    const std::vector<TnProblem> dec = {dp2, dp0};
    const bool dec_grouped = tn_set_groupable(dec, prec);
    if (!dec_grouped) PFN_TRY(launch_tn_set({dp2}, Mt, prec, det, lsc, NO_PROF, s, false));
    PFN_TRY(decoder_backward_data(m, w.dlog_t, w.dpre, w.dd_t, w.dxt, Mt));
    PFN_TRY(launch_tn_set(dec_grouped ? dec : std::vector<TnProblem>{dp0}, Mt, prec, det, lsc, NO_PROF, s, dec_grouped));
  }
  if (top_mode) {}
  else if (rg) PFN_TRY(launch_scatter_test_rows_ragged(dxt, d->nlayers > 0 ? (void*)w.gA_t : (void*)w.gA, S, B, E, rg->sep_of, (const long*)rg->row_off, d->nlayers > 0 ? prec : PFN_PREC_F32, s));
  else PFN_TRY(launch_scatter_test_rows(dxt, d->nlayers > 0 ? (void*)w.gA_t : (void*)w.gA, S, B, E, sep, d->nlayers > 0 ? prec : PFN_PREC_F32, s));

  auto view = [&](int l, bool compact) {
    const LayerP& p = L.layer[l];
    LayerWs& a = w.layer[l];
    float *db2 = pdrop > 0.f ? nullptr : grads + p.b2, *dbo = pdrop > 0.f ? nullptr : grads + p.b_o;
    return LayerGrads{compact ? (const void*)dxt : (const void*)w.gA_t, compact ? 0 : 1, a.y2, a.mean2, a.rstd2, params + p.g2, a.y1, a.mean1, a.rstd1, params + p.g1, a.hpre,
                      a.dy2_t, a.dy2m_t, a.dh_t, compact ? w.top_dy1_t : a.dy1_t, a.dqkv_t, w.gA_t,
                      LnSinks{grads + p.g2, grads + p.be2, db2}, LnSinks{grads + p.g1, grads + p.be1, dbo}, w.ln_part};
  };
  const bool emb_t = emb_gemm(*d, dsrc_sbe != nullptr);
  const bool fuse_lnb = d->nlayers > 0 && lnbwd_fusable(m, pl, lsc, view(0, false), M);
  auto launch_weight_gradients = [&](int l_hi, int l_lo) -> int {
    std::vector<TnProblem> probs, probs_top;
    auto add = [&](const void* A, long lda, const void* Bm, long ldb, float* C, long ldc, int P, int Q, float* colsum, bool compact = false) {
      TnProblem t; memset(&t, 0, sizeof(t)); t.A = A; t.lda = lda; t.B = Bm; t.ldb = ldb; t.C = C; t.ldc = ldc; t.P = P; t.Q = Q; t.colsum = colsum;
      (compact ? probs_top : probs).push_back(t);
    };
    for (int l = l_hi; l >= l_lo; --l) {
      const LayerP& p = L.layer[l];
      LayerWs& a = w.layer[l];
      const char* xin_t = (l == 0) ? w.x0_t : w.layer[l - 1].x2_t;
      const bool drop = pdrop > 0.f;
      const bool top = top_mode && l == d->nlayers - 1;
      add(drop ? a.dy2m_t : a.dy2_t, E, a.h, F, grads + p.w2, F, E, F, (drop || (fuse_lnb && l < d->nlayers - 1)) ? grads + p.b2 : nullptr, top);
      add(a.dh_t, F, a.x1_t, E, grads + p.w1, E, F, E, grads + p.b1, top);
      add(drop ? a.dy1m_t : (top ? w.top_dy1_t : a.dy1_t), E, top ? w.top_ctx_t : a.ctx, E, grads + p.w_o, E, E, E, (drop || fuse_lnb) ? grads + p.b_o : nullptr, top);
      add(a.dqkv_t, 3 * E, xin_t, E, grads + p.w_in, E, 3 * E, E, grads + p.b_in);
    }
    PFN_TRY(launch_tn_set(probs_top, Mt, prec, det, lsc, PFN_PROF_WGRAD + 1, s));
    PFN_TRY(launch_tn_set(probs, M, prec, det, lsc, PFN_PROF_WGRAD, s));
    return PFN_OK;
  };
  const int split_at = (on_first_group && first_group_layers > 0 && first_group_layers < d->nlayers) ? d->nlayers - first_group_layers : -1;
  bool delta_zeroed = false;
  for (int l = d->nlayers - 1; l >= 0; --l) {
    const LayerP& t = L.layer_t[l];
    LayerWs& a = w.layer[l];
    const bool top = top_mode && l == d->nlayers - 1;
    const int Ml = top ? Mt : M;
    char* dy1_t = top ? w.top_dy1_t : a.dy1_t;
    PFN_TRY(layer_backward_to_dy1(m, t, view(l, top), Ml, pl, fuse_lnb, fuse_lnb && l < d->nlayers - 1, lsc, pdrop, dseed(l, 3), top ? 1 : 0));
    const char* dy1_op = dy1_t;
    bool delta_fused = false;
    if (pdrop > 0.f) { PFN_TRY(launch_dropout_scale(a.dy1_t, a.dy1m_t, nullptr, nullptr, M, E, dseed(l, 1), pdrop, prec, s)); dy1_op = a.dy1m_t; }
    {
      ProfScope ps(PFN_PROF_GEMM_DCTX + (top ? 1 : 0), s);
      GemmNT g = nt(dy1_op, E, WT(m, t.w_o), E, Ml, E, E, EPI_OUT_T);
      g.out_t = top ? w.top_dctx_t : w.dctx_t; g.ld_out_t = E;
      if (!top && !det && g_fuse_delta) {
        GemmNT gd = g;
        gd.flags |= EPI_ROWDOT; gd.aux = a.ctx; gd.ld_aux = E;
        gd.rowdot = w.delta; gd.rd_lse = a.lse; gd.rd_lse2_off = (long)B * H * S; gd.rd_S = S; gd.rd_H = H; gd.rd_D = E / H;
        if (gemm_nt_rowdot_fused(gd, prec)) {
          if (!delta_zeroed && hipMemsetAsync(w.delta, 0, sizeof(float) * B * H * S, s) != hipSuccess) return fail(PFN_ERR_LAUNCH, "hipMemsetAsync(delta)");
          delta_zeroed = true;
          g = gd; delta_fused = true;
        }
      }
      PFN_TRY(launch_gemm_nt(g, prec, s));
    }
    if (top) {
      if (rg) {
        PFN_TRY(launch_scatter_rows_ragged(w.top_dctx_t, w.dctx_t, S, B, (long)E * es, rg->sep_of, (const long*)rg->row_off, 1, s));
        PFN_TRY(launch_scatter_rows_ragged(w.top_dy1_t, a.dy1_t, S, B, (long)E * es, rg->sep_of, (const long*)rg->row_off, 0, s));
      } else {
        PFN_TRY(launch_scatter_rows(w.top_dctx_t, w.dctx_t, S, B, (long)E * es, sep, sep / 256 * 256, s));
        PFN_TRY(launch_scatter_rows(w.top_dy1_t, a.dy1_t, S, B, (long)E * es, sep, 0, s));
      }
    }
    {
      AttnArgs at; memset(&at, 0, sizeof(at));
      at.qkv = a.qkv; at.ctx = a.ctx; at.lse = a.lse; at.B = B; at.S = S; at.E = E; at.H = H; at.sep = sep; at.sep_of = sep_of;
      at.dctx = w.dctx_t; at.dqkv = a.dqkv_t; at.delta = w.delta; at.ds = w.ds;
      at.p_drop = pdrop; at.drop_seed = dseed(l, 0);
      at.q_begin = top ? (rg ? rg->sep_min : sep) : 0;
      at.q_from_sep = (top && rg) ? 1 : 0;
      if (delta_fused) at.parts = ATTN_BWD_KV | ATTN_BWD_DQ;
      at.zero_delta = delta_zeroed ? 1 : 0;
      PFN_TRY(launch_attn_bwd(at, prec, s));
    }
    const LayerGrads below = l > 0 ? view(l - 1, false) : LayerGrads{};
    PFN_TRY(layer_backward_dx(m, t, a.dqkv_t, a.dy1_t, M, pl, lsc, fuse_lnb && l > 0 ? &below : nullptr, w.gA, w.gA_t, l == 0 && !emb_t, 0));
    if (l == split_at) {
      PFN_TRY(launch_weight_gradients(d->nlayers - 1, split_at));
      on_first_group(user);
    }
  }
  if (d->nlayers > 0) PFN_TRY(launch_weight_gradients(split_at >= 0 ? split_at - 1 : d->nlayers - 1, 0));
  const int aug = emb_aug_width(d->num_features);
  if (dsrc_sbe) {
    PFN_TRY(launch_bse_to_sbe(w.gA, dsrc_sbe, S, B, E, s, lsc));
  } else if (emb_t) {
    if (hipMemsetAsync(w.embacc, 0, sizeof(float) * E * aug, s) != hipSuccess) return fail(PFN_ERR_LAUNCH, "memset");
    GemmTN g = tn(w.gA_t, E, w.xaug_t, aug, w.embacc, aug, M, E, aug, grads + L.enc_b);
    g.scale_amax = lsc;
    g.max_splits = det ? 1 : 128;
    PFN_TRY(launch_gemm_tn(g, prec, s));
    PFN_TRY(launch_embed_grad_scatter(w.embacc, grads + L.enc_w, grads + L.yenc_w, grads + L.yenc_b, E, d->num_features, prec == PFN_PREC_FP16 ? w.xaug_amax : nullptr, s));
  } else {
    EmbedBwdArgs e;
    e.dsrc = w.gA; e.x = x; e.x_st = x_st; e.x_sb = x_sb; e.y = y; e.y_st = y_st; e.y_sb = y_sb;
    e.dwx = grads + L.enc_w; e.dbx = grads + L.enc_b; e.dwy = grads + L.yenc_w; e.dby = grads + L.yenc_b;
    e.S = S; e.B = B; e.nf = d->num_features; e.E = E; e.sep = sep; e.sep_of = sep_of; e.single_block = det ? 1 : 0; e.scale_amax = lsc;
    PFN_TRY(launch_embed_bwd(e, s));
  }
  return PFN_OK;
}

int pfn_stack_input_grads(const pfn_model_desc* d, const float* params, int B, int S, int sep, const void* workspace, int64_t workspace_bytes,
                          float* dx, int64_t dx_st, int64_t dx_sb, float* dy, int64_t dy_st, int64_t dy_sb, void* stream) {
  PFN_TRY(check_desc(d));
  if (B < 1 || S < 1 || sep < 0 || sep > S) return fail(PFN_ERR_ARGUMENT, "bad B=%d S=%d sep=%d", B, S, sep);
  if (!params || !workspace || !dx) return fail(PFN_ERR_ARGUMENT, "null pointer");
  Ws w = carve(*d, B, S, (char*)workspace);
  if (workspace_bytes < w.bytes) return fail(PFN_ERR_ARGUMENT, "workspace too small: %lld < %lld", (long long)workspace_bytes, (long long)w.bytes);
  const int prec = d->precision, E = d->emsize;
  const Layout L = make_layout(*d);
  hipStream_t s = (hipStream_t)stream;
  const bool emb_t = emb_gemm(*d, false);
  EmbedInGradArgs e; memset(&e, 0, sizeof(e));
  e.dsrc = emb_t ? (const void*)w.gA_t : (const void*)w.gA; e.dsrc_prec = emb_t ? prec : PFN_PREC_F32;
  e.wx = params + L.enc_w; e.wy = params + L.yenc_w;
  e.dx = dx; e.dx_st = dx_st; e.dx_sb = dx_sb; e.dy = dy; e.dy_st = dy_st; e.dy_sb = dy_sb;
  e.S = S; e.B = B; e.nf = d->num_features; e.E = E; e.sep = sep;
  e.scale_amax = (prec == PFN_PREC_FP16 && sep < S) ? w.lscale : nullptr;
  return launch_embed_input_grad(e, s);
}

int pfn_bar_mean_backward(const float* logits, int64_t ld, const float* borders, int64_t R, int nbars, int full_support, const float* mean, const float* gout,
                          float* dlogits, void* stream) {
  if (R < 0 || nbars < 1 || (R > 0 && (!logits || !borders || !mean || !gout || !dlogits))) return fail(PFN_ERR_ARGUMENT, "bad bar_mean_backward arguments");
  BarArgs a; memset(&a, 0, sizeof(a));
  a.logits = logits; a.ld = ld; a.borders = borders; a.R = R; a.nbars = nbars; a.full_support = full_support;
  a.mean_out = const_cast<float*>(mean); a.gout = gout; a.dlogits = dlogits;
  PFN_TRY(launch_bar_mean_bwd(a, (hipStream_t)stream));
  return PFN_OK;
}

int pfn_bar_nll_forward(const float* logits, int64_t ld, const float* y, const float* borders, int64_t R, int nbars,
                        int full_support, float* nll, float* lse, int32_t* bucket, void* stream) {
  if (R < 0 || nbars < 1 || (R > 0 && (!logits || !y || !borders || !nll || !lse || !bucket))) return fail(PFN_ERR_ARGUMENT, "bad bar_nll_forward arguments");
  BarArgs a; memset(&a, 0, sizeof(a));
  a.logits = logits; a.ld = ld; a.y = y; a.borders = borders; a.R = R; a.nbars = nbars; a.full_support = full_support;
  a.nll = nll; a.lse = lse; a.bucket = bucket;
  PFN_TRY(launch_bar_nll_fwd(a, (hipStream_t)stream));
  return PFN_OK;
}
int pfn_bar_nll_backward(const float* logits, int64_t ld, const float* lse, const int32_t* bucket, const float* gout,
                         int64_t R, int nbars, float* dlogits, void* stream) {
  if (R < 0 || nbars < 1 || (R > 0 && (!logits || !lse || !bucket || !gout || !dlogits))) return fail(PFN_ERR_ARGUMENT, "bad bar_nll_backward arguments");
  BarArgs a; memset(&a, 0, sizeof(a));
  a.logits = logits; a.ld = ld; a.R = R; a.nbars = nbars; a.lse = const_cast<float*>(lse); a.bucket = const_cast<int*>(bucket);
  a.gout = gout; a.dlogits = dlogits;
  PFN_TRY(launch_bar_nll_bwd(a, (hipStream_t)stream));
  return PFN_OK;
}
int pfn_bar_mean(const float* logits, int64_t ld, const float* borders, int64_t R, int nbars, int full_support, float* mean, void* stream) {
  if (R < 0 || nbars < 1 || (R > 0 && (!logits || !borders || !mean))) return fail(PFN_ERR_ARGUMENT, "bad bar_mean arguments");
  BarArgs a; memset(&a, 0, sizeof(a));
  a.logits = logits; a.ld = ld; a.borders = borders; a.R = R; a.nbars = nbars; a.full_support = full_support; a.mean_out = mean;
  PFN_TRY(launch_bar_mean(a, (hipStream_t)stream));
  return PFN_OK;
}

static int bar_stats_common(BarStatsArgs& a, const char* what, const float* logits, int64_t ld, const float* borders, int64_t R, int nbars, int full_support) {
  if (R < 0) return fail(PFN_ERR_ARGUMENT, "%s: R = %lld", what, (long long)R);
  if (nbars < 1 || (full_support && nbars < 2)) return fail(PFN_ERR_ARGUMENT, "%s: nbars = %d%s", what, nbars, full_support ? " (full support needs two buckets)" : "");
  if (ld < nbars) return fail(PFN_ERR_ARGUMENT, "%s: ld %lld < nbars %d", what, (long long)ld, nbars);
  if (!logits || !borders) return fail(PFN_ERR_ARGUMENT, "%s: null pointer", what);
  memset(&a, 0, sizeof(a));
  a.logits = logits; a.ld = ld; a.borders = borders; a.R = R; a.nbars = nbars; a.full_support = full_support ? 1 : 0;
  return PFN_OK;
// ... 241 lines not shown
  const int64_t need = bnn_svgd_workspace_bytes(P, num_particles, D);
  if (workspace_bytes < need || (need > 0 && !workspace))
    return fail(PFN_ERR_ARGUMENT, "workspace_bytes %lld < pfn_bnn_svgd_workspace_bytes = %lld (or a NULL workspace)", (long long)workspace_bytes, (long long)need);
  if (num_steps == 0) return PFN_OK;
  BnnSvgdArgs a{};
  a.x = x; a.y = y; a.n_of = n_of; a.state = state; a.ld = ld; a.P = P; a.S = S; a.F = F; a.H = H; a.activation = activation; a.N = num_particles; a.step0 = step0;
  a.num_steps = num_steps; a.lr = lr; a.beta1 = beta1; a.beta2 = beta2; a.eps = eps; a.bandwidth_factor = bandwidth_factor;
  a.grads = need > 0 ? (float*)workspace : nullptr; a.potential = potential; a.bandwidth = bandwidth;
  PFN_TRY(launch_bnn_svgd_steps(a, (hipStream_t)stream));
  return PFN_OK;
}

int pfn_mlp_prior_forward(const float* weights, const float* biases, const int32_t* model_of, const int32_t* dims, const float* noise_std,
                          float* causes, const float* noise, float* y, float* hidden, int B, int T, int HP, int Lmax, int activation, int gen_causes,
                          uint64_t seed, uint64_t offset, void* stream) {
  if (!weights || !biases || !model_of || !dims || !noise_std || !causes || !y) return fail(PFN_ERR_ARGUMENT, "bad mlp_prior_forward arguments");
  if (activation < 0 || activation > 3) return fail(PFN_ERR_UNSUPPORTED, "activation %d (0 identity, 1 relu, 2 tanh, 3 sigmoid)", activation);
  MlpPriorArgs a;
  a.weights = weights; a.biases = biases; a.model_of = model_of; a.dims = dims; a.noise_std = noise_std; a.causes = causes; a.noise = noise; a.y = y; a.hidden = hidden;
  a.B = B; a.T = T; a.HP = HP; a.Lmax = Lmax; a.activation = activation; a.gen_causes = gen_causes; a.seed = seed; a.offset = offset;
  PFN_TRY(launch_mlp_prior(a, (hipStream_t)stream));
  return PFN_OK;
}

int pfn_op_gemm_nt(const void* A, int64_t lda, const void* B, int64_t ldb, int M, int N, int K, int flags, const float* bias,
                   const void* aux, int64_t ld_aux, const float* resid, int64_t ld_resid, float* out_f32, int64_t ld_out_f32,
                   void* out_t, int64_t ld_out_t, void* out2_t, int64_t ld_out2, int prec, void* stream) {
  GemmNT g = nt(A, lda, B, ldb, M, N, K, flags);
  g.bias = bias; g.aux = aux; g.ld_aux = ld_aux; g.resid = resid; g.ld_resid = ld_resid; g.out_f32 = out_f32; g.ld_out_f32 = ld_out_f32;
  g.out_t = out_t; g.ld_out_t = ld_out_t; g.out2_t = out2_t; g.ld_out2 = ld_out2;
  PFN_TRY(launch_gemm_nt(g, prec, (hipStream_t)stream));
  return PFN_OK;
}
int pfn_op_gemm_tn(const void* A, int64_t lda, const void* B, int64_t ldb, float* C, int64_t ldc, int M, int P, int Q, int atomic, int prec, void* stream) {
  GemmTN g = tn(A, lda, B, ldb, C, ldc, M, P, Q);
  g.atomic = atomic;
  PFN_TRY(launch_gemm_tn(g, prec, (hipStream_t)stream));
  return PFN_OK;
}
int pfn_op_gemm_tn_group(int n, const void* const* A, const int64_t* lda, const void* const* B, const int64_t* ldb, float* const* C,
                         const int64_t* ldc, const int32_t* P, const int32_t* Q, float* const* colsum, int M, int splits, int prec, void* stream) {
  if (n < 1 || n > TN_GROUP_MAX || !A || !lda || !B || !ldb || !C || !ldc || !P || !Q) return fail(PFN_ERR_ARGUMENT, "bad gemm_tn_group arguments");
  GemmTNGroup g;
  memset(&g, 0, sizeof(g));
  g.n = n; g.M = M; g.splits = splits;
  for (int i = 0; i < n; ++i) {
    TnProblem& t = g.p[i];
    t.A = A[i]; t.lda = lda[i]; t.B = B[i]; t.ldb = ldb[i]; t.C = C[i]; t.ldc = ldc[i]; t.P = P[i]; t.Q = Q[i];
    t.colsum = colsum ? colsum[i] : nullptr;
  }
  PFN_TRY(launch_gemm_tn_group(g, prec, (hipStream_t)stream));
  return PFN_OK;
}
int pfn_op_gemm_ln(const void* A, int64_t lda, const void* B, int64_t ldb, int M, int N, int K, const float* bias,
                   const float* resid, const float* ry, const float* rmean, const float* rrstd, const float* rgamma, const float* rbeta,
                   const float* gamma, const float* beta, float eps, float* y, float* mean, float* rstd, void* x_t, int prec, void* stream) {
  GemmLN g;
  memset(&g, 0, sizeof(g));
  g.A = A; g.lda = lda; g.B = B; g.ldb = ldb; g.M = M; g.N = N; g.K = K; g.bias = bias; g.resid = resid;
  g.ry = ry; g.rmean = rmean; g.rrstd = rrstd; g.rgamma = rgamma; g.rbeta = rbeta; g.gamma = gamma; g.beta = beta; g.eps = eps;
  g.y = y; g.mean = mean; g.rstd = rstd; g.x_t = x_t; g.y16 = (prec & PFN_OP_SUMS_16BIT) ? 1 : 0;
  PFN_TRY(launch_gemm_ln(g, prec & ~PFN_OP_SUMS_16BIT, (hipStream_t)stream));
  return PFN_OK;
}
int pfn_op_gemm_lnbwd(const void* A, int64_t lda, const void* B, int64_t ldb, int M, int N, int K, const void* aux,
                      const float* y, const float* mean, const float* rstd, const float* gamma,
                      void* dx_t, float* dgamma, float* dbeta, int prec, void* stream) {
  GemmLNB g;
  memset(&g, 0, sizeof(g));
  g.A = A; g.lda = lda; g.B = B; g.ldb = ldb; g.M = M; g.N = N; g.K = K; g.aux = aux;
  g.y = y; g.mean = mean; g.rstd = rstd; g.gamma = gamma; g.dx_t = dx_t; g.dgamma = dgamma; g.dbeta = dbeta; g.y16 = (prec & PFN_OP_SUMS_16BIT) ? 1 : 0;
  PFN_TRY(launch_gemm_lnbwd(g, prec & ~PFN_OP_SUMS_16BIT, (hipStream_t)stream));
  return PFN_OK;
}
int pfn_op_attention_fwd(const void* qkv, void* ctx, float* lse, int B, int S, int E, int H, int sep, int prec, void* stream) {
  AttnArgs at; memset(&at, 0, sizeof(at));
  at.qkv = qkv; at.ctx = ctx; at.lse = lse; at.B = B; at.S = S; at.E = E; at.H = H; at.sep = sep;
  PFN_TRY(launch_attn_fwd(at, prec, (hipStream_t)stream));
  return PFN_OK;
}
int pfn_op_attention_fwd_from(const void* qkv, void* ctx, float* lse, int B, int S, int E, int H, int sep, int q_begin, int prec, void* stream) {
  AttnArgs at; memset(&at, 0, sizeof(at));
  at.qkv = qkv; at.ctx = ctx; at.lse = lse; at.B = B; at.S = S; at.E = E; at.H = H; at.sep = sep; at.q_begin = q_begin;
  PFN_TRY(launch_attn_fwd(at, prec, (hipStream_t)stream));
  return PFN_OK;
}
int pfn_op_attention_bwd_from(const void* qkv, const void* ctx, const float* lse, const void* dctx, void* dqkv, float* delta_ws, void* ds_ws,
                              int B, int S, int E, int H, int sep, int q_begin, int prec, int parts, void* stream) {
  AttnArgs at; memset(&at, 0, sizeof(at));
  at.qkv = qkv; at.ctx = const_cast<void*>(ctx); at.lse = const_cast<float*>(lse); at.B = B; at.S = S; at.E = E; at.H = H; at.sep = sep;
  at.dctx = dctx; at.dqkv = dqkv; at.delta = delta_ws; at.ds = ds_ws; at.parts = parts; at.q_begin = q_begin;
  PFN_TRY(launch_attn_bwd(at, prec, (hipStream_t)stream));
  return PFN_OK;
}
int pfn_op_gather_rows(const void* src_bs, void* dst_tb, int B, int S, int64_t row_bytes, int sep, void* stream) {
  if (!src_bs || !dst_tb || B < 1 || S < 1 || sep < 0 || sep > S) return fail(PFN_ERR_ARGUMENT, "bad gather_rows arguments");
  PFN_TRY(launch_gather_rows(src_bs, dst_tb, S, B, row_bytes, sep, (hipStream_t)stream));
  return PFN_OK;
}
int pfn_op_scatter_rows(const void* src_tb, void* dst_bs, int B, int S, int64_t row_bytes, int sep, int zero_from, void* stream) {
  if (!src_tb || !dst_bs || B < 1 || S < 1 || sep < 0 || sep > S) return fail(PFN_ERR_ARGUMENT, "bad scatter_rows arguments");
  PFN_TRY(launch_scatter_rows(src_tb, dst_bs, S, B, row_bytes, sep, zero_from, (hipStream_t)stream));
  return PFN_OK;
}
int64_t pfn_op_attention_bwd_ws_bytes(int B, int S, int H, int prec) {
  if (B < 1 || S < 1 || H < 1) return -1;
// ... 40 lines not shown
```

transformerscandobayesianinference_amd/csrc/pfn_kernels.h:

```cpp
#pragma once
#include <hip/hip_runtime.h>
#include <stdint.h>
#include <atomic>
#include "../../include/pfn_hip.h"

namespace pfn {

struct LdsAllowance {
  std::atomic<size_t> granted[16];
  template <typename K> void ensure(K kernel, size_t bytes) {
    int dev = 0;
    (void)hipGetDevice(&dev);
    std::atomic<size_t>& g = granted[dev & 15];
    if (bytes <= g.load(std::memory_order_acquire)) return;
    (void)hipFuncSetAttribute(reinterpret_cast<const void*>(kernel), hipFuncAttributeMaxDynamicSharedMemorySize, (int)bytes);
    size_t cur = g.load(std::memory_order_relaxed);
    while (cur < bytes && !g.compare_exchange_weak(cur, bytes, std::memory_order_release)) {}
  }
};

inline bool prec_is16(int p) { return p == PFN_PREC_BF16 || p == PFN_PREC_FP16; }
inline int prec_esize(int p) { return prec_is16(p) ? 2 : 4; }
#define PFN_DISPATCH_OP(prec, ...)                                                          \
  do {                                                                                      \
// ... 36 lines not shown
  EPI_GELU = 2,
  EPI_GELU_BWD = 4,
  EPI_RESID = 8,
  EPI_OUT_F32 = 16,
  EPI_OUT_T = 32,
  EPI_OUT2_T = 64,
  EPI_ACCUM = 128,
  EPI_RESID_T = 256,
  EPI_ROWDOT = 512,
  EPI_ROWSHIFT = 1024,
};

struct GemmNT {
  const void* A; long lda;
  const void* B; long ldb;
  int M, N, K;
  int flags;
  const float* bias;
  const void* aux; long ld_aux;
  const float* resid; long ld_resid;
  float* out_f32; long ld_out_f32;
  void* out_t; long ld_out_t;
  void* out2_t; long ld_out2;
  int vec_ok;
  int wide_t;
  float* rowdot; const float* rd_lse; long rd_lse2_off; int rd_S, rd_H, rd_D;
  const float* rowshift; long rs_ld; int rs_S, rs_n0, rs_n1;
};
int launch_key_shift(const void* x_t, const void* w_k_t, float* kshift, int B, int S, int E, int sep, const int* sep_of, int precision, hipStream_t s);
int launch_gemm_nt(const GemmNT& g, int precision, hipStream_t stream);
bool gemm_nt_rowdot_fused(const GemmNT& g, int precision);
void set_gemm_nt_big_mode(int mode);
void set_gemm_ln_rows64(int on);

struct GemmTN {
  const void* A; long lda;
  const void* B; long ldb;
  float* C; long ldc;
  int M, P, Q;
  int atomic;
  int m_chunk;
  float* colsum;
  int max_splits;
  const float* scale_amax;
};
int launch_gemm_tn(GemmTN g, int precision, hipStream_t stream);

constexpr int TN_GROUP_MAX = 26;
struct TnProblem {
  const void* A; const void* B; float* C; float* colsum;
  long lda, ldb, ldc;
  int P, Q;
  int Pv;
};
struct GemmTNGroup {
  TnProblem p[TN_GROUP_MAX];
  int tile_start[TN_GROUP_MAX + 1];
  int n, M, splits, m_chunk;
  int debug_mask;
  const float* scale_amax;
};
void set_gemm_tn_debug_wrap(int rows);
void set_gemm_tn_group_waves(int waves);
void set_gemm_tn_group_splits(int splits);
struct GemmLN {
  const void* A; long lda;
  const void* B; long ldb;
  int M, N, K;
  const float* bias;
  const float* resid;
  const void* ry; const float* rmean; const float* rrstd; const float* rgamma; const float* rbeta;
  const float* gamma; const float* beta; float eps;
  void* y; float* mean; float* rstd; void* x_t;
  float* x_f32;
  int y16;
};
bool gemm_ln_supported(const GemmLN& g);
int launch_gemm_ln(const GemmLN& g, int precision, hipStream_t stream);

struct GemmLNB {
  const void* A; long lda;
  const void* B; long ldb;
  int M, N, K;
  const void* aux;
  const void* y; const float* mean; const float* rstd; const float* gamma;
  void* dx_t;
  float* dgamma; float* dbeta;
  const float* scale_amax;
  int y16;
};
bool gemm_lnbwd_supported(const GemmLNB& g);
int launch_gemm_lnbwd(const GemmLNB& g, int precision, hipStream_t stream);

bool gemm_tn_group_supported(const TnProblem& p);
int launch_gemm_tn_group(GemmTNGroup g, int precision, hipStream_t stream);

struct AttnArgs {
  const void* qkv; void* ctx; float* lse;
  int B, S, E, H, sep;
  const int* sep_of;
  int q_from_sep;
  union {
    struct {
      const void* dctx; void* dqkv; float* delta;
      void* ds;
      int ds_rows, ds_ld;
      int parts;
      int zero_delta;
    };
    struct {
      const void* kv; long kv_ld, kv_sb;
      float* part_o;
      float* part_ml;
      int split_keys;
    };
  };
  int pingpong;
  int b0, bg;
  const void* xq;
  const void* wq;
  const float* bq;
  int q_store;
  int q_begin;
  float p_drop;
  unsigned drop_seed;
};
int attn_cache_splits(int B, int n, int E, int H, int sep, int precision);
int launch_attn_fwd_cache(const AttnArgs& a, int precision, hipStream_t stream);
void set_attn_cache_split_cap(int splits);
struct AttnCacheBwdArgs {
  const void* qkv;
  const void* ctx;
  const float* lse;
  const void* dctx;
  void* dqkv;
  const void* kv; long kv_ld, kv_sb;
  float* part_dq;
  int B, S, E, H, sep;
  int split_keys;
  const int* sep_of;
};
int launch_clamp_sep_of(const int* src, int* dst, int B, int hi, hipStream_t stream);
int launch_attn_bwd_cache(const AttnCacheBwdArgs& a, int precision, hipStream_t stream);
void set_attn_pingpong(int mask);
void set_attn_bwd_group(int datasets);
enum : int { ATTN_BWD_DELTA = 1, ATTN_BWD_KV = 2, ATTN_BWD_DQ = 4 };
int64_t attn_bwd_ds_bytes(int B, int S, int H, int precision);
int launch_attn_fwd(const AttnArgs& a, int precision, hipStream_t stream);
bool attn_fwd_can_fuse_q(int E, int H, int precision);
int launch_attn_bwd(const AttnArgs& a, int precision, hipStream_t stream);

int launch_cast_params(const float* src, void* dst_t, long n, int precision, hipStream_t s);
constexpr int TRANSPOSE_GROUP_MAX = 64;
struct TransposeGroup {
  int n = 0, blocks = 0;
  long src_off[TRANSPOSE_GROUP_MAX], dst_off[TRANSPOSE_GROUP_MAX];
  int rows[TRANSPOSE_GROUP_MAX], cols[TRANSPOSE_GROUP_MAX], ld_dst[TRANSPOSE_GROUP_MAX], first_block[TRANSPOSE_GROUP_MAX];
};
void transpose_group_add(TransposeGroup& g, long src_off, long dst_off, int rows, int cols, int ld_dst);
int launch_transpose_cast_group(const float* src, void* dst, const TransposeGroup& g, int precision, hipStream_t s);
int launch_transpose_cast(const float* src, void* dst_t, int rows, int cols, long ld_dst, int precision, hipStream_t s);
int launch_cast_rows(const float* src, long ld_src, void* dst_t, long ld_dst, long R, int C, int precision, hipStream_t s, const float* scale_amax = nullptr);
int launch_absmax(const float* x, long n, float* amax, hipStream_t s);
int set_loss_scale_target(int log2_target);
int launch_scale_copy(const float* src, float* dst, long n, const float* scale_amax, hipStream_t s);

struct EmbedArgs {
  const float* x; long x_st, x_sb;
  const float* y; long y_st, y_sb;
  const float* wx; const float* bx;
  const float* wy; const float* by;
  float* out_f32; void* out_t;
  void* xaug_t;
  int xaug_ld;
  const float* xaug_amax;
  int S, B, nf, E, sep;
  const int* sep_of;
};
constexpr int EMB_MAX_FEATURES = 1022;
__host__ __device__ inline int emb_aug_width(int nf) { return nf + 2 <= 32 ? 32 : nf + 2 <= 64 ? 64 : nf + 2 <= 128 ? 128 : 0; }
int launch_embed_fwd(const EmbedArgs& a, int precision, hipStream_t s);
int launch_embed_colmax(const EmbedArgs& a, float* amax, hipStream_t s);
__device__ inline int xaug_col_exp(const float* amax, int f) {
  if (!amax) return 0;
  const float m = amax[f];
  if (!(m > 0.f) || !(m <= 3.402823466e38f)) return 0;
  const int e = ilogbf(m);
  return e < -126 ? -126 : e;
}
struct EmbedBwdArgs {
  const float* dsrc; const float* x; long x_st, x_sb; const float* y; long y_st, y_sb;
  float* dwx; float* dbx; float* dwy; float* dby;
  int S, B, nf, E, sep;
  const int* sep_of;
  int single_block;
  const float* scale_amax;
};
int launch_embed_bwd(const EmbedBwdArgs& a, hipStream_t s);
int launch_embed_grad_scatter(const float* acc, float* dwx, float* dwy, float* dby, int E, int nf, const float* xaug_amax, hipStream_t s);
struct EmbedInGradArgs {
  const void* dsrc; int dsrc_prec;
  const float* wx; const float* wy;
  float* dx; long dx_st, dx_sb;
  float* dy; long dy_st, dy_sb;
  int S, B, nf, E, sep;
  const float* scale_amax;
};
int launch_embed_input_grad(const EmbedInGradArgs& a, hipStream_t s);

int launch_sbe_to_bse(const float* src, float* out_f32, void* out_t, int S, int B, int E, int precision, hipStream_t s);
int launch_bse_to_sbe(const float* src_bse, float* dst_sbe, int S, int B, int E, hipStream_t s, const float* scale_amax = nullptr);

int launch_layernorm_fwd(const void* x, const float* gamma, const float* beta, float* y_f32, void* y_t,
                         float* mean, float* rstd, long rows, int E, float eps, int precision, hipStream_t s, int x_is_t = 0);
int launch_layernorm_bwd(const void* dy, int dy_is_t, const void* x, const float* gamma, const float* mean, const float* rstd,
                         float* dx_f32, void* dx_t, float* dgamma, float* dbeta, float* dbias_extra,
                         long rows, int E, int precision, hipStream_t s, float* partials = nullptr, const float* scale_amax = nullptr, int x_is_t = 0);
constexpr int LNB_MAX_BLOCKS = 512;
int launch_colsum(const void* a_t, long lda, long rows, int cols, float* out, int precision, hipStream_t s);

int launch_dropout_add(float* y, const float* resid, long rows, int cols, unsigned site_seed, float p, hipStream_t s);
int launch_dropout_scale(const void* src, void* dst, const void* src2, void* dst2, long rows, int cols, unsigned site_seed, float p, int precision, hipStream_t s);
int launch_gather_test_rows(const float* src_bse, void* dst_t, int S, int B, int E, int sep, int precision, hipStream_t s);
int launch_gather_rows_ragged(const void* src_bs, void* dst, int S, int B, long row_bytes, const int* sep_of, const long* row_off, hipStream_t s);
int launch_scatter_rows_ragged(const void* src, void* dst_bs, int S, int B, long row_bytes, const int* sep_of, const long* row_off, int zero_from_block, hipStream_t s);
int launch_zero_row_prefix_ragged(void* base, int S, int B, const int* sep_of, long row_bytes, long width_bytes, hipStream_t s);
int launch_gather_test_rows_ragged(const float* src_bse, void* dst_t, int S, int B, int E, const int* sep_of, const long* row_off, int precision, hipStream_t s);
int launch_scatter_test_rows_ragged(const float* src, void* dst_bse_t, int S, int B, int E, const int* sep_of, const long* row_off, int precision, hipStream_t s);
int launch_scatter_test_rows(const float* src, void* dst_bse_t, int S, int B, int E, int sep, int precision, hipStream_t s);
int launch_gather_rows(const void* src_bs, void* dst_tb, int S, int B, long row_bytes, int sep, hipStream_t s);
int launch_scatter_rows(const void* src_tb, void* dst_bs, int S, int B, long row_bytes, int sep, int zero_from, hipStream_t s);
int launch_zero_row_prefix(void* base, int S, int B, int nrows, long row_bytes, long width_bytes, hipStream_t s);

struct BarArgs {
  const float* logits; long ld;
  const float* y;
  const float* borders;
  float* nll;
  float* lse;
  int* bucket;
  long R; int nbars; int full_support;
  const float* gout; float* dlogits;
  float* mean_out;
};
int launch_bar_nll_fwd(const BarArgs& a, hipStream_t s);
int launch_bar_nll_bwd(const BarArgs& a, hipStream_t s);
int launch_bar_mean(const BarArgs& a, hipStream_t s);
int launch_bar_mean_bwd(const BarArgs& a, hipStream_t s);
struct BarStatsArgs {
  const float* logits; long ld;
  const float* borders;
  long R; int nbars; int full_support;
// ... 150 lines not shown
```

transformerscandobayesianinference_amd/csrc/rowwise.hip:

```cpp
#include <algorithm>
#include "pfn_device.h"
#include "pfn_kernels.h"

namespace pfn {

template <typename T> PFN_DEV void st4(T* p, f32x4 x) {
  if constexpr (sizeof(T) == 2) {
    X4<T> v;
#pragma unroll
    for (int e = 0; e < 4; ++e) v[e] = (T)x[e];
    *reinterpret_cast<X4<T>*>(p) = v;
  } else *reinterpret_cast<f32x4*>(p) = x;
}
template <typename T> PFN_DEV f32x4 ld4(const T* p) {
  f32x4 r;
  if constexpr (sizeof(T) == 2) {
    X4<T> v = *reinterpret_cast<const X4<T>*>(p);
#pragma unroll
    for (int e = 0; e < 4; ++e) r[e] = (float)v[e];
  } else r = *reinterpret_cast<const f32x4*>(p);
  return r;
}

static int grid_for(long work_items, int per_block, int cap = 4096) {
// ... 159 lines not shown
    }
#pragma unroll
    for (int e = 0; e < 8; ++e) part[rl * E + cg * 8 + e] = acc[e];
  }
  __syncthreads();
  const float inv = 1.f / (float)ns;
  for (int e = threadIdx.x; e < E; e += 256) {
    float s = 0.f;
    for (int rl = 0; rl < R; ++rl) s += part[rl * E + e];
    part[e] = s * inv;
  }
  __syncthreads();
  const int wave = threadIdx.x >> 6, lane = threadIdx.x & 63;
  for (int pass = 0; pass * 512 < E; ++pass) {
    const int e0 = pass * 512 + lane * 8;
    const bool live = e0 < E;
    const int ec = live ? e0 : 0;
    X8<T> w[16];
#pragma unroll
    for (int o = 0; o < 16; ++o) w[o] = *reinterpret_cast<const X8<T>*>(wk + (long)min(n0 + wave * 16 + o, E - 1) * E + ec);
    float xv[8];
#pragma unroll
    for (int e = 0; e < 8; ++e) xv[e] = live ? part[ec + e] : 0.f;
#pragma unroll
    for (int o = 0; o < 16; ++o) {
      float s = 0.f;
#pragma unroll
      for (int e = 0; e < 8; ++e) s += (float)w[o][e] * xv[e];
      s = wave_sum(s);
      const int n = n0 + wave * 16 + o;
      if (lane == 0 && n < E) {
        if (pass == 0) kshift[(long)b * E + n] = s;
        else kshift[(long)b * E + n] += s;
      }
    }
  }
}
int launch_key_shift(const void* x_t, const void* w_k_t, float* kshift, int B, int S, int E, int sep, const int* sep_of, int precision, hipStream_t s) {
  if (!prec_is16(precision) || E % 8 || E > 2048 || B < 1 || S < 1) return PFN_ERR_UNSUPPORTED;
  const dim3 grid((E + 63) / 64, B);
  if (precision == PFN_PREC_FP16) hipLaunchKernelGGL(key_shift_kernel<f16>, grid, dim3(256), 0, s, (const f16*)x_t, (const f16*)w_k_t, kshift, S, E, sep, sep_of);
  else hipLaunchKernelGGL(key_shift_kernel<bf16>, grid, dim3(256), 0, s, (const bf16*)x_t, (const bf16*)w_k_t, kshift, S, E, sep, sep_of);
  return PFN_LAUNCH_OK();
}

constexpr int EMB_TOK = 16;
template <typename T> __global__ __launch_bounds__(256) void embed_fwd_kernel(EmbedArgs a) {
  operand_store_mode<T>();
  extern __shared__ float xs[];
  __shared__ int xexp[128];
  const long ntok = (long)a.B * a.S;
  const long t0 = (long)blockIdx.x * EMB_TOK;
  const int nfp = a.nf + 2;
  if (a.xaug_t && threadIdx.x < a.xaug_ld) xexp[threadIdx.x] = xaug_col_exp(a.xaug_amax, threadIdx.x);
  for (int i = threadIdx.x; i < EMB_TOK * nfp; i += 256) {
    const int tk = i / nfp, f = i % nfp;
    const long tok = t0 + tk;
    float v = 0.f;
    if (tok < ntok) {
      const long b = tok / a.S, sidx = tok % a.S;
      const int sep = a.sep_of ? a.sep_of[b] : a.sep;
      if (f < a.nf) v = a.x[sidx * a.x_st + b * a.x_sb + f];
      else if (f == a.nf) v = (sidx < sep) ? a.y[sidx * a.y_st + b * a.y_sb] : 0.f;
      else v = (sidx < sep) ? 1.f : 0.f;
    }
    xs[i] = v;
  }
  __syncthreads();
  T* out_t = reinterpret_cast<T*>(a.out_t);
  if (a.xaug_t) {
    T* xa = reinterpret_cast<T*>(a.xaug_t);
    const int aug = a.xaug_ld;
    for (int i = threadIdx.x; i < EMB_TOK * aug; i += 256) {
      const int tk = i / aug, f = i % aug;
      if (t0 + tk < ntok) xa[(t0 + tk) * aug + f] = (T)(f < nfp ? ldexpf(xs[tk * nfp + f], -xexp[f]) : 0.f);
    }
  }
  for (int e = threadIdx.x; e < a.E; e += 256) {
    const float be = a.bx[e], wye = a.wy[e], bye = a.by[e];
    float acc[EMB_TOK];
#pragma unroll
    for (int tk = 0; tk < EMB_TOK; ++tk) acc[tk] = __builtin_fmaf(xs[tk * nfp + a.nf + 1], bye, __builtin_fmaf(xs[tk * nfp + a.nf], wye, be));
    for (int f = 0; f < a.nf; ++f) {
      const float w = a.wx[(long)e * a.nf + f];
#pragma unroll
      for (int tk = 0; tk < EMB_TOK; ++tk) acc[tk] = __builtin_fmaf(w, xs[tk * nfp + f], acc[tk]);
    }
#pragma unroll
    for (int tk = 0; tk < EMB_TOK; ++tk) {
      const long tok = t0 + tk;
      if (tok < ntok) {
        a.out_f32[tok * a.E + e] = acc[tk];
        out_t[tok * a.E + e] = (T)acc[tk];
      }
    }
  }
}
__global__ __launch_bounds__(256) void embed_colmax_kernel(EmbedArgs a, unsigned* amax_bits) {
  __shared__ unsigned cm[128];
  if (threadIdx.x < 128) cm[threadIdx.x] = 0u;
  __syncthreads();
  const long ntok = (long)a.B * a.S;
  const int nfy = a.nf + 1;
  const long i0 = (long)blockIdx.x * 256 + threadIdx.x, stride = (long)gridDim.x * 256 / nfy * nfy;
  if (i0 < stride) {
    const int f = (int)(i0 % nfy);
    float m = 0.f;
    for (long i = i0; i < ntok * nfy; i += stride) {
      const long tok = i / nfy, b = tok / a.S, sidx = tok % a.S;
      const int sep = a.sep_of ? a.sep_of[b] : a.sep;
      m = fmaxf(m, fabsf(f < a.nf ? a.x[sidx * a.x_st + b * a.x_sb + f] : ((sidx < sep) ? a.y[sidx * a.y_st + b * a.y_sb] : 0.f)));
    }
    if (m > 0.f) atomicMax(cm + f, __builtin_bit_cast(unsigned, m));
  }
  __syncthreads();
  if (threadIdx.x < nfy && cm[threadIdx.x]) atomicMax(amax_bits + threadIdx.x, cm[threadIdx.x]);
}
int launch_embed_colmax(const EmbedArgs& a, float* amax, hipStream_t s) {
  if (a.xaug_ld <= 0 || a.xaug_ld > 128 || a.nf + 2 > a.xaug_ld) return PFN_ERR_UNSUPPORTED;
  if (hipMemsetAsync(amax, 0, sizeof(float) * a.xaug_ld, s) != hipSuccess) return PFN_ERR_LAUNCH;
  const long n = (long)a.B * a.S * (a.nf + 1);
  hipLaunchKernelGGL(embed_colmax_kernel, dim3(grid_for(n, 256 * 16, 1024)), dim3(256), 0, s, a, reinterpret_cast<unsigned*>(amax));
  return PFN_LAUNCH_OK();
}
int launch_embed_fwd(const EmbedArgs& a, int precision, hipStream_t s) {
// ... 81 lines not shown
  float acc[8] = {0.f, 0.f, 0.f, 0.f, 0.f, 0.f, 0.f, 0.f};
  float db = 0.f;
  for (long t0 = tbeg; t0 < tend; t0 += EMBW_TOK) {
    __syncthreads();
    for (int i = threadIdx.x; i < EMBW_TOK * 8; i += 256) {
      const int tk = i >> 3, f = f0 + (i & 7);
      const long tok = t0 + tk;
      float v = 0.f;
      if (tok < tend) {
        const long b = tok / a.S, sidx = tok % a.S;
        const int sep = a.sep_of ? a.sep_of[b] : a.sep;
        if (f < a.nf) v = a.x[sidx * a.x_st + b * a.x_sb + f];
        else if (f == a.nf) v = (sidx < sep) ? a.y[sidx * a.y_st + b * a.y_sb] : 0.f;
        else if (f == a.nf + 1) v = (sidx < sep) ? 1.f : 0.f;
      }
      xs[i] = v;
    }
    __syncthreads();
    if (e >= a.E) continue;
    const int ntk = (int)std::min<long>(EMBW_TOK, tend - t0);
    for (int tk = 0; tk < ntk; ++tk) {
      const float d = a.dsrc[(t0 + tk) * a.E + e];
      db += d;
      const f32x4 x0 = *reinterpret_cast<const f32x4*>(xs + tk * 8), x1 = *reinterpret_cast<const f32x4*>(xs + tk * 8 + 4);
#pragma unroll
      for (int q = 0; q < 4; ++q) { acc[q] += d * x0[q]; acc[4 + q] += d * x1[q]; }
    }
  }
  if (e >= a.E) return;
  const float osc = loss_scale_down(a.scale_amax);
#pragma unroll
  for (int j = 0; j < 8; ++j) {
    const int f = f0 + j;
    if (f < a.nf) unsafeAtomicAdd(a.dwx + (long)e * a.nf + f, acc[j] * osc);
    else if (f == a.nf) unsafeAtomicAdd(a.dwy + e, acc[j] * osc);
    else if (f == a.nf + 1) unsafeAtomicAdd(a.dby + e, acc[j] * osc);
  }
  if (blockIdx.y == 0) unsafeAtomicAdd(a.dbx + e, db * osc);
}
__global__ __launch_bounds__(256) void embed_grad_scatter_kernel(const float* acc, float* dwx, float* dwy, float* dby, int E, int nf, const float* xaug_amax) {
  const int i = blockIdx.x * 256 + threadIdx.x;
  if (i >= E * (nf + 2)) return;
  const int e = i / (nf + 2), f = i % (nf + 2);
  const float v = ldexpf(acc[e * emb_aug_width(nf) + f], xaug_col_exp(xaug_amax, f));
  if (f < nf) unsafeAtomicAdd(dwx + (long)e * nf + f, v);
  else if (f == nf) unsafeAtomicAdd(dwy + e, v);
  else unsafeAtomicAdd(dby + e, v);
}
int launch_embed_grad_scatter(const float* acc, float* dwx, float* dwy, float* dby, int E, int nf, const float* xaug_amax, hipStream_t s) {
  if (emb_aug_width(nf) == 0) return PFN_ERR_UNSUPPORTED;
  hipLaunchKernelGGL(embed_grad_scatter_kernel, dim3((E * (nf + 2) + 255) / 256), dim3(256), 0, s, acc, dwx, dwy, dby, E, nf, xaug_amax);
  return PFN_LAUNCH_OK();
}
__global__ __launch_bounds__(256) void embed_input_grad_kernel(EmbedInGradArgs a, int R, int fc) {
  extern __shared__ float eig_sm[];
  float* ds = eig_sm;
  float* wt = eig_sm + (long)R * a.E;
  const int E = a.E, WS = E + 1;
  const long M = (long)a.B * a.S, m0 = (long)blockIdx.x * R;
  const int nr = (int)std::min<long>(R, M - m0);
  const float osc = loss_scale_down(a.scale_amax);
  for (int i = threadIdx.x; i < nr * E; i += 256) {
    const long k = m0 * E + i;
    float v;
    if (a.dsrc_prec == PFN_PREC_F32) v = reinterpret_cast<const float*>(a.dsrc)[k];
    else if (a.dsrc_prec == PFN_PREC_BF16) v = (float)reinterpret_cast<const bf16*>(a.dsrc)[k];
    else v = (float)reinterpret_cast<const f16*>(a.dsrc)[k];
    ds[i] = v * osc;
  }
  __syncthreads();
  const int g = threadIdx.x >> 4, l16 = threadIdx.x & 15;
  auto sum16 = [](float v) {
#pragma unroll
    for (int off = 8; off > 0; off >>= 1) v += __shfl_xor(v, off, 64);
    return v;
  };
  if (a.dy) {
    for (int r = g; r < nr; r += 16) {
      const long m = m0 + r, b = m / a.S, t = m % a.S;
      float v = 0.f;
      if (t < a.sep)
        for (int e = l16; e < E; e += 16) v += ds[r * E + e] * a.wy[e];
      v = sum16(v);
      if (l16 == 0) a.dy[t * a.dy_st + b * a.dy_sb] = v;
    }
  }
  for (int f0 = 0; f0 < a.nf; f0 += fc) {
    const int nfc = min(fc, a.nf - f0);
    __syncthreads();
    for (int i = threadIdx.x; i < nfc * E; i += 256) {
      const int e = i / nfc, j = i - e * nfc;
      wt[j * WS + e] = a.wx[(long)e * a.nf + f0 + j];
    }
    __syncthreads();
    for (int p = g; p < nr * nfc; p += 16) {
      const int r = p / nfc, j = p - r * nfc;
      float v = 0.f;
      for (int e = l16; e < E; e += 16) v += ds[r * E + e] * wt[j * WS + e];
      v = sum16(v);
      const long m = m0 + r, b = m / a.S, t = m % a.S;
      if (l16 == 0) a.dx[t * a.dx_st + b * a.dx_sb + f0 + j] = v;
    }
  }
}
int launch_embed_input_grad(const EmbedInGradArgs& a, hipStream_t s) {
  const long M = (long)a.B * a.S;
// ... 548 lines not shown
```

transformerscandobayesianinference_amd/hipops.py:

```python
import ctypes
import math

import torch

from transformerscandobayesianinference_amd import _hip

TDT = {_hip.PREC_BF16: torch.bfloat16, _hip.PREC_F32: torch.float32, _hip.PREC_FP16: torch.float16}
PREC_OF = {v: k for k, v in TDT.items()}
MANGLED_OPERAND = {_hip.PREC_BF16: 'DF16b', _hip.PREC_FP16: 'DF16_', _hip.PREC_F32: 'f'}


def sp():
    return _hip.stream_ptr()


def gemm_nt(A, B, flags, prec, bias=None, aux=None, resid=None, out_f32=None, out_t=None, out2_t=None):
    M, K = A.shape
    N = B.shape[0]
    p = _hip.ptr
    ld = lambda t: 0 if t is None else t.stride(0)
    _hip.check(_hip.lib().pfn_op_gemm_nt(p(A), A.stride(0), p(B), B.stride(0), M, N, K, flags, p(bias), p(aux), ld(aux),
                                         p(resid), ld(resid), p(out_f32), ld(out_f32), p(out_t), ld(out_t), p(out2_t), ld(out2_t),
                                         prec, sp()), 'pfn_op_gemm_nt')


def gemm_tn(A, B, C, prec, atomic=1):
    M, P = A.shape
    Q = B.shape[1]
    _hip.check(_hip.lib().pfn_op_gemm_tn(A.data_ptr(), A.stride(0), B.data_ptr(), B.stride(0), C.data_ptr(), C.stride(0), M, P, Q,
                                         atomic, prec, sp()), 'pfn_op_gemm_tn')


def gemm_tn_group(problems, splits=0):
    import ctypes
    n = len(problems)
    M = problems[0][0].shape[0]
    VP, L, I = ctypes.c_void_p * n, ctypes.c_int64 * n, ctypes.c_int32 * n
    A = VP(*[p[0].data_ptr() for p in problems]); lda = L(*[p[0].stride(0) for p in problems])
    B = VP(*[p[1].data_ptr() for p in problems]); ldb = L(*[p[1].stride(0) for p in problems])
    C = VP(*[p[2].data_ptr() for p in problems]); ldc = L(*[p[2].stride(0) for p in problems])
    P = I(*[p[0].shape[1] for p in problems]); Q = I(*[p[1].shape[1] for p in problems])
    cs = VP(*[(p[3].data_ptr() if p[3] is not None else None) for p in problems])
    _hip.check(_hip.lib().pfn_op_gemm_tn_group(n, A, lda, B, ldb, C, ldc, P, Q, cs, M, splits, PREC_OF[problems[0][0].dtype], sp()), 'pfn_op_gemm_tn_group')


SUMS_16BIT = 256


def gemm_ln(A, B, bias, gamma, beta, eps, resid=None, prev=None, out=None, sums16=False):
    M, K = A.shape
    N = B.shape[0]
    dev = A.device
    if out is None:
        y = torch.full((M + 2, N), float('nan'), dtype=A.dtype if sums16 else torch.float32, device=dev)
        x_t = torch.empty(M, N, dtype=A.dtype, device=dev)
        mean, rstd = torch.empty(M, device=dev), torch.empty(M, device=dev)
    else:
        y, x_t, mean, rstd = out
    p = _hip.ptr
    pv = prev if prev is not None else (None,) * 5
    assert y.dtype == (A.dtype if sums16 else torch.float32) and (pv[0] is None or pv[0].dtype == y.dtype)
    _hip.check(_hip.lib().pfn_op_gemm_ln(p(A), A.stride(0), p(B), B.stride(0), M, N, K, p(bias), p(resid), p(pv[0]), p(pv[1]), p(pv[2]), p(pv[3]), p(pv[4]),
                                         p(gamma), p(beta), eps, p(y), p(mean), p(rstd), p(x_t), PREC_OF[A.dtype] | (SUMS_16BIT if sums16 else 0), sp()), 'pfn_op_gemm_ln')
    if out is None:
        assert torch.isnan(y[M:]).all()
    return y[:M], x_t, mean, rstd


def attention_fwd(qkv, H, sep, prec, q_begin=0, out=None):
    B, S, E3 = qkv.shape
    E = E3 // 3
    if q_begin:
        if out is not None:
            ctx, lse = out
        else:
            ctx = torch.full((B, S, E), float('nan'), dtype=qkv.dtype, device=qkv.device)
            lse = torch.full((B, H, S), float('nan'), dtype=torch.float32, device=qkv.device)
        _hip.check(_hip.lib().pfn_op_attention_fwd_from(qkv.data_ptr(), ctx.data_ptr(), lse.data_ptr(), B, S, E, H, sep, q_begin, prec, sp()), 'attn fwd')
        return ctx, lse
    ctx = torch.empty(B, S, E, dtype=qkv.dtype, device=qkv.device)
    lse = torch.empty(B, H, S, dtype=torch.float32, device=qkv.device)
    _hip.check(_hip.lib().pfn_op_attention_fwd(qkv.data_ptr(), ctx.data_ptr(), lse.data_ptr(), B, S, E, H, sep, prec, sp()), 'attn fwd')
    return ctx, lse


def gather_rows(src, sep, out=None):
    B, S, W = src.shape
    dst = out if out is not None else torch.empty((S - sep) * B, W, dtype=src.dtype, device=src.device)
    _hip.check(_hip.lib().pfn_op_gather_rows(src.data_ptr(), dst.data_ptr(), B, S, W * src.element_size(), sep, sp()), 'gather rows')
    return dst


def scatter_rows(src, B, S, sep, zero_from, fill=float('nan'), out=None):
    W = src.shape[1]
    dst = out if out is not None else torch.full((B, S, W), fill, dtype=src.dtype, device=src.device)
    _hip.check(_hip.lib().pfn_op_scatter_rows(src.data_ptr(), dst.data_ptr(), B, S, W * src.element_size(), sep, zero_from, sp()), 'scatter rows')
# ... 297 lines not shown
```

transformerscandobayesianinference_amd/transformer.py:

```python
import ctypes

import torch
from torch import nn

from transformerscandobayesianinference_amd import _hip
from transformerscandobayesianinference_amd.positional_encodings import NoPositionalEncoding
from transformerscandobayesianinference_amd.utils import SeqBN

_ALIGN = 64


class _SelfAttentionParams(nn.Module):

    def __init__(self, emsize):
        super().__init__()
        self.in_proj_weight = nn.Parameter(torch.empty(3 * emsize, emsize))
        self.in_proj_bias = nn.Parameter(torch.zeros(3 * emsize))
        self.out_proj = nn.Linear(emsize, emsize)
        nn.init.xavier_uniform_(self.in_proj_weight)
        nn.init.zeros_(self.out_proj.bias)


class _EncoderLayerParams(nn.Module):

# ... 32 lines not shown
            if x.dtype != torch.float32 or x.stride(-1) != 1:
                x = x.float().contiguous()
            if y.dtype != torch.float32:
                y = y.float()
            S, B = x.shape[0], x.shape[1]
            x_ptr, y_ptr = x.data_ptr(), y.data_ptr()
            x_st, x_sb = x.stride(0), x.stride(1)
            y_st, y_sb = y.stride(0), y.stride(1)
        ws_bytes = lib.pfn_workspace_bytes(ctypes.byref(desc), B, S)
        _hip.check(ws_bytes, 'pfn_workspace_bytes')
        ws = torch.empty(ws_bytes, dtype=torch.uint8, device=dev)
        ctx.ragged = ragged
        if ragged is not None:
            sep_of, row_off, sep_min, sep_max, test_rows = ragged
            logits = torch.empty((test_rows, desc.n_out or desc.emsize), dtype=torch.float32, device=dev)
            ctx.dropout_seed = model._next_dropout_seed() if (model.training and desc.dropout > 0) else None
            _hip.check(lib.pfn_stack_forward_ragged(ctypes.byref(desc), flat_params.data_ptr(), shadow.data_ptr(), x_ptr, x_st, x_sb, y_ptr, y_st, y_sb, B, S,
                                                    sep_of.data_ptr(), row_off.data_ptr(), sep_min, sep_max, test_rows, ws.data_ptr(), ws_bytes, logits.data_ptr(), stream,
                                                    int(ctx.dropout_seed is not None), ctx.dropout_seed or 0), 'pfn_stack_forward_ragged')
            ctx.model, ctx.ws, ctx.dims = model, ws, (B, S, sep_max)
            ctx.operands = (desc, shadow)
            ctx.inputs = (x, y, None)
            ctx.src_needs_grad = False
            return logits
        logits = torch.empty((S - sep, B, desc.n_out or desc.emsize), dtype=torch.float32, device=dev)
        ctx.dropout_seed = None
        if model.training and desc.dropout > 0:
            ctx.dropout_seed = model._next_dropout_seed()
            _hip.check(lib.pfn_stack_forward_dropout(ctypes.byref(desc), flat_params.data_ptr(), shadow.data_ptr(),
                                                     x_ptr, x_st, x_sb, y_ptr, y_st, y_sb, _hip.ptr(src), B, S, sep,
                                                     ws.data_ptr(), ws_bytes, logits.data_ptr(), stream, ctx.dropout_seed), 'pfn_stack_forward_dropout')
        else:
            _hip.check(lib.pfn_stack_forward(ctypes.byref(desc), flat_params.data_ptr(), shadow.data_ptr(),
                                             x_ptr, x_st, x_sb, y_ptr, y_st, y_sb, _hip.ptr(src), B, S, sep,
                                             ws.data_ptr(), ws_bytes, logits.data_ptr(), stream), 'pfn_stack_forward')
        ctx.model, ctx.ws, ctx.dims = model, ws, (B, S, sep)
        ctx.operands = (desc, shadow)
        ctx.inputs = (x, y, src)
        ctx.src_needs_grad = src is not None and ctx.needs_input_grad[4]
        return logits

    @staticmethod
    def backward(ctx, dlogits):
        lib = _hip.lib()
        model, ws = ctx.model, ctx.ws
        B, S, sep = ctx.dims
        x, y, src = ctx.inputs
        dev = ws.device
        stream = _hip.stream_ptr(dev)
        desc, shadow = ctx.operands
        if desc is not model._desc:
            raise RuntimeError('backward through an inference-precision forward: the forward of this graph ran the eval_precision kernels')
        model._attach_grads()
        dlogits = dlogits.contiguous().float()
        dsrc = None
        if src is not None:
            dsrc = torch.empty_like(src)
            args = (0, 0, 0, 0, 0, 0)
        else:
            args = (x.data_ptr(), x.stride(0), x.stride(1), y.data_ptr(), y.stride(0), y.stride(1))
        hook = model._first_group_hook
        split = hook is not None and hook.armed()
        if ctx.ragged is not None:
            sep_of, row_off, sep_min, sep_max, test_rows = ctx.ragged
            cb = _hip.HOST_CALLBACK(lambda user: hook.first_group_launched()) if split else None
            _hip.check(lib.pfn_stack_backward_ragged(ctypes.byref(desc), model._flat.data_ptr(), shadow.data_ptr(), *args, B, S,
                                                     sep_of.data_ptr(), row_off.data_ptr(), sep_min, sep_max, test_rows, ws.data_ptr(), ws.numel(), dlogits.data_ptr(),
                                                     model._flat_grad.data_ptr(), stream, hook.first_group_layers if split else 0, cb, None,
                                                     int(ctx.dropout_seed is not None), ctx.dropout_seed or 0), 'pfn_stack_backward_ragged')
            ctx.ws = None
            return None, None, None, None, None, None, None, None
        if split or ctx.dropout_seed is not None:
            cb = _hip.HOST_CALLBACK(lambda user: hook.first_group_launched()) if split else None
            _hip.check(lib.pfn_stack_backward_split(ctypes.byref(desc), model._flat.data_ptr(), shadow.data_ptr(), *args,
                                                    B, S, sep, ws.data_ptr(), ws.numel(), dlogits.data_ptr(),
                                                    model._flat_grad.data_ptr(), _hip.ptr(dsrc), stream,
                                                    hook.first_group_layers if split else 0, cb, None,
                                                    int(ctx.dropout_seed is not None), ctx.dropout_seed or 0),
                       'pfn_stack_backward_split')
        else:
            _hip.check(lib.pfn_stack_backward(ctypes.byref(desc), model._flat.data_ptr(), shadow.data_ptr(), *args,
                                              B, S, sep, ws.data_ptr(), ws.numel(), dlogits.data_ptr(),
                                              model._flat_grad.data_ptr(), _hip.ptr(dsrc), stream), 'pfn_stack_backward')
        dx = dy = None
        if src is None and (ctx.needs_input_grad[2] or ctx.needs_input_grad[3]):
            dx = torch.empty((S, B, x.shape[2]), dtype=torch.float32, device=dev)
            dy = torch.empty((S, B), dtype=torch.float32, device=dev) if ctx.needs_input_grad[3] else None
            if sep == S:
                dx.zero_()
                if dy is not None:
                    dy.zero_()
            else:
                _hip.check(lib.pfn_stack_input_grads(ctypes.byref(desc), model._flat.data_ptr(), B, S, sep, ws.data_ptr(), ws.numel(),
                                                     dx.data_ptr(), dx.stride(0), dx.stride(1), _hip.ptr(dy), B, 1, stream),
                           'pfn_stack_input_grads')
        ctx.ws = None
        return (None, None, dx if ctx.needs_input_grad[2] else None, dy, (dsrc if ctx.src_needs_grad else None), None, None, None)


class _PredictFunction(torch.autograd.Function):

    @staticmethod
    def forward(ctx, x, model, context, desc, shadow):
        lib = _hip.lib()
        dev = x.device
        stream = _hip.stream_ptr(dev)
# ... 478 lines not shown
```

Baseline: 2574 datasets/s.

## Compute embedding weight grads from first-layer wgrad via grouped TN GEMM with per-problem rows

Adds a path where the embedding encoder's weight gradient is derived algebraically from the first layer's input-projection weight-gradient GEMM outputs, using a 256-pitched xaug buffer and a new finish kernel, instead of materializing dsrc. It also generalizes the grouped TN GEMM to per-problem row counts and per-problem chunk planning with a CU-aware cost model. The aim is to skip a separate embedding backward pass and to balance wave rounds better. It costs extra workspace and an extra reduction kernel with atomics, and it is bypassed when input grads are needed or determinism is requested.

After: 2586 datasets/s, median of 6. No clear change (+0.5%).

```diff
diff --git a/include/pfn_hip.h b/include/pfn_hip.h
--- a/include/pfn_hip.h
+++ b/include/pfn_hip.h
@@ -41,6 +41,7 @@
        PFN_SCHED_KEY_CENTERING = 64,
        PFN_SCHED_F32_RESIDUAL = 128,
        PFN_SCHED_FUSE_Q_PROJECTION = 32,
+       PFN_SCHED_KEEP_DSRC = 256,
        PFN_SCHED_DETERMINISTIC = 8        };
 int pfn_default_schedule(void);
 
@@ -262,6 +263,11 @@
 int pfn_op_gemm_tn_group(int n, const void* const* A, const int64_t* lda, const void* const* B, const int64_t* ldb,
                          float* const* C, const int64_t* ldc, const int32_t* P, const int32_t* Q,
                          float* const* colsum, int M, int splits, int prec, void* stream);
+int pfn_op_gemm_tn_group_rows(int n, const void* const* A, const int64_t* lda, const void* const* B, const int64_t* ldb,
+                              float* const* C, const int64_t* ldc, const int32_t* P, const int32_t* Q,
+                              float* const* colsum, const int32_t* M, int splits, int prec, void* stream);
+int pfn_op_gemm_tn_group_plan(int n, const int32_t* P, const int32_t* Q, const int32_t* M, int splits, int cus,
+                              int32_t* chunks, int32_t* chunk_rows);
 #define PFN_OP_SUMS_16BIT 256
 int pfn_op_gemm_ln(const void* A, int64_t lda, const void* B, int64_t ldb, int M, int N, int K, const float* bias,
                    const float* resid, const float* ry, const float* rmean, const float* rrstd,
diff --git a/transformerscandobayesianinference_amd/_hip.py b/transformerscandobayesianinference_amd/_hip.py
--- a/transformerscandobayesianinference_amd/_hip.py
+++ b/transformerscandobayesianinference_amd/_hip.py
@@ -13,7 +13,7 @@
 PREC_F32 = 1
 PREC_FP16 = 2
 PRECISIONS = {'bf16': PREC_BF16, 'f32': PREC_F32, 'fp32': PREC_F32, 'fp16': PREC_FP16, 'f16': PREC_FP16}
-SCHED_TOP_LAYER_ALL_ROWS, SCHED_FUSE_LN_WIDE, SCHED_SEPARATE_LNBWD, SCHED_DETERMINISTIC, SCHED_NO_KEY_CENTERING, SCHED_FUSE_Q_PROJECTION, SCHED_KEY_CENTERING, SCHED_F32_RESIDUAL = 1, 2, 4, 8, 16, 32, 64, 128
+SCHED_TOP_LAYER_ALL_ROWS, SCHED_FUSE_LN_WIDE, SCHED_SEPARATE_LNBWD, SCHED_DETERMINISTIC, SCHED_NO_KEY_CENTERING, SCHED_FUSE_Q_PROJECTION, SCHED_KEY_CENTERING, SCHED_F32_RESIDUAL, SCHED_KEEP_DSRC = 1, 2, 4, 8, 16, 32, 64, 128, 256
 NUTS_ADAPT_MASS, NUTS_KEEP_WARMUP, NUTS_MAX_WINDOWS, NUTS_INV_MASS_OFFSET = 1, 2, 16, 256
 
 EPI_BIAS, EPI_GELU, EPI_GELU_BWD, EPI_RESID, EPI_OUT_F32, EPI_OUT_T, EPI_OUT2_T, EPI_ACCUM, EPI_RESID_T = 1, 2, 4, 8, 16, 32, 64, 128, 256
@@ -97,6 +97,8 @@
     'pfn_op_gemm_nt': (_I, [_P, _L, _P, _L, _I, _I, _I, _I, _P, _P, _L, _P, _L, _P, _L, _P, _L, _P, _L, _I, _P]),
     'pfn_op_gemm_tn': (_I, [_P, _L, _P, _L, _P, _L, _I, _I, _I, _I, _I, _P]),
     'pfn_op_gemm_tn_group': (_I, [_I, _P, _P, _P, _P, _P, _P, _P, _P, _P, _I, _I, _I, _P]),
+    'pfn_op_gemm_tn_group_rows': (_I, [_I, _P, _P, _P, _P, _P, _P, _P, _P, _P, _P, _I, _I, _P]),
+    'pfn_op_gemm_tn_group_plan': (_I, [_I, _P, _P, _P, _I, _I, _P, _P]),
     'pfn_op_gemm_ln': (_I, [_P, _L, _P, _L, _I, _I, _I, _P, _P, _P, _P, _P, _P, _P, _P, _P, _F, _P, _P, _P, _P, _I, _P]),
     'pfn_op_gemm_lnbwd': (_I, [_P, _L, _P, _L, _I, _I, _I, _P, _P, _P, _P, _P, _P, _P, _P, _I, _P]),
     'pfn_op_attention_fwd': (_I, [_P, _P, _P, _I, _I, _I, _I, _I, _I, _P]),
diff --git a/transformerscandobayesianinference_amd/csrc/gemm_tn.hip b/transformerscandobayesianinference_amd/csrc/gemm_tn.hip
--- a/transformerscandobayesianinference_amd/csrc/gemm_tn.hip
+++ b/transformerscandobayesianinference_amd/csrc/gemm_tn.hip
@@ -1,3 +1,4 @@
+#include <algorithm>
 #include <type_traits>
 #include "pfn_device.h"
 #include "pfn_kernels.h"
@@ -185,23 +186,32 @@
   }
 };
 
+struct TnItem { int pi, p0, q0, rows; long mbeg; };
+PFN_DEV TnItem tn_item(const GemmTNGroup& g, int bid) {
+  const int id = xcd_remap(bid, g.item_start[g.n]);
+  TnItem it;
+  it.pi = 0;
+  while (id >= g.item_start[it.pi + 1]) ++it.pi;
+  const TnProblem& pr = g.p[it.pi];
+  const int tq = pr.Q / 256, tiles = (pr.P / 256) * tq;
+  const int local = id - g.item_start[it.pi];
+  const int chunk = local / tiles, tl = local % tiles;
+  it.p0 = (tl / tq) * 256; it.q0 = (tl % tq) * 256;
+  it.mbeg = (long)chunk * g.chunk[it.pi];
+  it.rows = (int)min((long)g.chunk[it.pi], pr.M - it.mbeg);
+  return it;
+}
+
 template <typename T>
 __global__ __launch_bounds__(512, 1) void gemm_tn_big_kernel(GemmTNGroup g) {
   extern __shared__ __attribute__((aligned(16))) char smem_raw[];
   LdsPtr smem = lds_cast(smem_raw);
 
-  const int ntiles = g.tile_start[g.n];
-  const int id = xcd_remap(blockIdx.x, ntiles * g.splits);
-  const int split = id / ntiles, tile = id % ntiles;
-  int pi = 0;
-  while (tile >= g.tile_start[pi + 1]) ++pi;
-  const TnProblem& pr = g.p[pi];
-  const int tq = pr.Q / 256;
-  const int tl = tile - g.tile_start[pi];
-  const int p0 = (tl / tq) * 256, q0 = (tl % tq) * 256;
-  const long mbeg = (long)split * g.m_chunk;
-  const long mend = min((long)g.M, mbeg + g.m_chunk);
-  const int rows_total = (int)(mend - mbeg);
+  const TnItem it = tn_item(g, blockIdx.x);
+  const TnProblem& pr = g.p[it.pi];
+  const int p0 = it.p0, q0 = it.q0;
+  const long mbeg = it.mbeg;
+  const int rows_total = it.rows;
   if (rows_total <= 0) return;
 
   const int wave = __builtin_amdgcn_readfirstlane(threadIdx.x >> 6), lane = threadIdx.x & 63;
@@ -307,18 +317,11 @@
 __global__ __launch_bounds__(TNW_NW * 64, 1) void gemm_tn_wide_kernel(GemmTNGroup g) {
   extern __shared__ __attribute__((aligned(16))) char smem_raw[];
   LdsPtr smem = lds_cast(smem_raw);
-  const int ntiles = g.tile_start[g.n];
-  const int id = xcd_remap(blockIdx.x, ntiles * g.splits);
-  const int split = id / ntiles, tile = id % ntiles;
-  int pi = 0;
-  while (tile >= g.tile_start[pi + 1]) ++pi;
-  const TnProblem& pr = g.p[pi];
-  const int tq = pr.Q / 256;
-  const int tl = tile - g.tile_start[pi];
-  const int p0 = (tl / tq) * 256, q0 = (tl % tq) * 256;
-  const long mbeg = (long)split * g.m_chunk;
-  const long mend = min((long)g.M, mbeg + g.m_chunk);
-  const int rows_total = (int)(mend - mbeg);
+  const TnItem it = tn_item(g, blockIdx.x);
+  const TnProblem& pr = g.p[it.pi];
+  const int p0 = it.p0, q0 = it.q0;
+  const long mbeg = it.mbeg;
+  const int rows_total = it.rows;
   if (rows_total <= 0) return;
   const int wave = __builtin_amdgcn_readfirstlane(threadIdx.x >> 6), lane = threadIdx.x & 63;
   const int wp = wave >> 1, wq = wave & 1;
@@ -452,36 +455,82 @@
   return p.P % 256 == 0 && p.Q % 256 == 0 && (p.lda * 2) % 16 == 0 && (p.ldb * 2) % 16 == 0 && aligned16(p.A) && aligned16(p.B);
 }
 
+static void tn_uniform_chunks(int M, int splits, int* chunks, int* chunk_rows) {
+  const int max_splits = (M + 4 * TNB_KT - 1) / (4 * TNB_KT);
+  if (splits > max_splits) splits = max_splits;
+  int chunk = (M + splits - 1) / splits;
+  chunk = (chunk + TNB_KT - 1) / TNB_KT * TNB_KT;
+  *chunks = (M + chunk - 1) / chunk;
+  *chunk_rows = chunk;
+}
+constexpr int TN_FLUSH_STAGES = 24;
+int tn_group_plan(int n, const int* P, const int* Q, const int* M, int splits, int cus, int* chunks, int* chunk_rows) {
+  if (cus <= 0) cus = 256;
+  auto items_of = [&]() { int it = 0; for (int i = 0; i < n; ++i) it += (P[i] / 256) * (Q[i] / 256) * chunks[i]; return it; };
+  int m_max = 0;
+  for (int i = 0; i < n; ++i) { chunks[i] = 0; chunk_rows[i] = TNB_KT; m_max = std::max(m_max, M[i]); }
+  if (m_max <= 0) return 0;
+  auto cut = [&](int sp) {
+    int c_max, rows_max;
+    tn_uniform_chunks(m_max, sp, &c_max, &rows_max);
+    const int T = rows_max / TNB_KT;
+    for (int i = 0; i < n; ++i) {
+      if (M[i] <= 0) { chunks[i] = 0; continue; }
+      if (splits > 0) { tn_uniform_chunks(M[i], sp, &chunks[i], &chunk_rows[i]); continue; }
+      const int stages = (M[i] + TNB_KT - 1) / TNB_KT;
+      tn_uniform_chunks(M[i], (stages + T - 1) / T, &chunks[i], &chunk_rows[i]);
+    }
+    return T;
+  };
+  if (splits > 0) { cut(splits); return items_of(); }
+  int best = 8;
+  long best_cost = -1;
+  for (int sp = 1; sp <= 8; ++sp) {
+    const int T = cut(sp), items = items_of(), rounds = (items + cus - 1) / cus;
+    if (items < 0.9 * rounds * cus) continue;
+    const long cost = (long)rounds * (T + TN_FLUSH_STAGES);
+    if (best_cost < 0 || cost < best_cost) { best_cost = cost; best = sp; }
+  }
+  cut(best);
+  return items_of();
+}
+
+static int device_cus() {
+  static int cus[64] = {0};
+  int dev = 0;
+  if (hipGetDevice(&dev) != hipSuccess || dev < 0 || dev >= 64) return 256;
+  if (cus[dev] == 0) {
+    int v = 0;
+    cus[dev] = (hipDeviceGetAttribute(&v, hipDeviceAttributeMultiprocessorCount, dev) == hipSuccess && v > 0) ? v : 256;
+  }
+  return cus[dev];
+}
+
 int launch_gemm_tn_group(GemmTNGroup g, int precision, hipStream_t stream) {
-  if (g.n <= 0 || g.M <= 0) return PFN_OK;
+  if (g.n <= 0) return PFN_OK;
   if (g.n > TN_GROUP_MAX) return PFN_ERR_ARGUMENT;
   if (!prec_is16(precision)) return PFN_ERR_UNSUPPORTED;
-  int tiles = 0;
+  int P[TN_GROUP_MAX], Q[TN_GROUP_MAX], M[TN_GROUP_MAX], chunks[TN_GROUP_MAX];
   for (int i = 0; i < g.n; ++i) {
     if (!gemm_tn_group_supported(g.p[i])) return PFN_ERR_UNSUPPORTED;
-    g.tile_start[i] = tiles;
-    tiles += (g.p[i].P / 256) * (g.p[i].Q / 256);
-  }
-  g.tile_start[g.n] = tiles;
+    P[i] = g.p[i].P; Q[i] = g.p[i].Q;
+    M[i] = g.p[i].M == 0 ? std::max(g.M, 0) : std::max(g.p[i].M, 0);
+    g.p[i].M = M[i];
+  }
   int splits = g.splits;
   if (splits <= 0 && g_tn_group_splits > 0) splits = g_tn_group_splits;
-  if (splits <= 0) {
-    splits = 8;
-    for (int sp = 1; sp <= 8; ++sp) {
-      const int blocks = tiles * sp, rounds = (blocks + 255) / 256;
-      if (blocks >= 0.9 * rounds * 256) { splits = sp; break; }
-    }
-  }
-  const int max_splits = (g.M + 4 * TNB_KT - 1) / (4 * TNB_KT);
-  if (splits > max_splits) splits = max_splits;
-  int chunk = (g.M + splits - 1) / splits;
-  chunk = (chunk + TNB_KT - 1) / TNB_KT * TNB_KT;
-  splits = (g.M + chunk - 1) / chunk;
-  g.splits = splits;
-  g.m_chunk = chunk;
+  const int items = tn_group_plan(g.n, P, Q, M, splits, splits > 0 ? 0 : device_cus(), chunks, g.chunk);
+  if (items <= 0) return PFN_OK;
+  int at = 0;
+  for (int i = 0; i < g.n; ++i) {
+    g.item_start[i] = at;
+    at += (P[i] / 256) * (Q[i] / 256) * chunks[i];
+  }
+  g.item_start[g.n] = at;
   for (int i = 0; i < g.n; ++i) {
     const TnProblem& p = g.p[i];
-    if (p.lda < 256 || p.ldb < 256 || (long)chunk * p.lda * 2 > TN_GROUP_MAX_SPLIT_BYTES || (long)chunk * p.ldb * 2 > TN_GROUP_MAX_SPLIT_BYTES) return PFN_ERR_UNSUPPORTED;
+    if (chunks[i] == 0) continue;
+    if (p.lda < 256 || p.ldb < 256 || (long)g.chunk[i] * p.lda * 2 > TN_GROUP_MAX_SPLIT_BYTES || (long)g.chunk[i] * p.ldb * 2 > TN_GROUP_MAX_SPLIT_BYTES) return PFN_ERR_UNSUPPORTED;
   }
   const int wrap = g_tn_debug_wrap;
   g.debug_mask = wrap >= TNB_KT && (wrap & (wrap - 1)) == 0 ? wrap - 1 : 0x7fffffff;
@@ -490,10 +539,10 @@
     static LdsAllowance allow_w[2];
     if (precision == PFN_PREC_FP16) {
       allow_w[1].ensure(gemm_tn_wide_kernel<f16>, TNB_LDS);
-      hipLaunchKernelGGL(gemm_tn_wide_kernel<f16>, dim3(tiles * splits), dim3(TNW_NW * 64), TNB_LDS, stream, g);
+      hipLaunchKernelGGL(gemm_tn_wide_kernel<f16>, dim3(items), dim3(TNW_NW * 64), TNB_LDS, stream, g);
     } else {
       allow_w[0].ensure(gemm_tn_wide_kernel<bf16>, TNB_LDS);
-      hipLaunchKernelGGL(gemm_tn_wide_kernel<bf16>, dim3(tiles * splits), dim3(TNW_NW * 64), TNB_LDS, stream, g);
+      hipLaunchKernelGGL(gemm_tn_wide_kernel<bf16>, dim3(items), dim3(TNW_NW * 64), TNB_LDS, stream, g);
     }
     return hipGetLastError() == hipSuccess ? PFN_OK : PFN_ERR_LAUNCH;
 #else
@@ -503,10 +552,10 @@
   static LdsAllowance allowance[2];
   if (precision == PFN_PREC_FP16) {
     allowance[1].ensure(gemm_tn_big_kernel<f16>, TNB_LDS);
-    hipLaunchKernelGGL(gemm_tn_big_kernel<f16>, dim3(tiles * splits), dim3(512), TNB_LDS, stream, g);
+    hipLaunchKernelGGL(gemm_tn_big_kernel<f16>, dim3(items), dim3(512), TNB_LDS, stream, g);
   } else {
     allowance[0].ensure(gemm_tn_big_kernel<bf16>, TNB_LDS);
-    hipLaunchKernelGGL(gemm_tn_big_kernel<bf16>, dim3(tiles * splits), dim3(512), TNB_LDS, stream, g);
+    hipLaunchKernelGGL(gemm_tn_big_kernel<bf16>, dim3(items), dim3(512), TNB_LDS, stream, g);
   }
   return hipGetLastError() == hipSuccess ? PFN_OK : PFN_ERR_LAUNCH;
 }
diff --git a/transformerscandobayesianinference_amd/csrc/pfn_api.hip b/transformerscandobayesianinference_amd/csrc/pfn_api.hip
--- a/transformerscandobayesianinference_amd/csrc/pfn_api.hip
+++ b/transformerscandobayesianinference_amd/csrc/pfn_api.hip
@@ -67,7 +67,7 @@
   const bool ok = dh == 32 || dh == 64 || dh == 128 || dh == 256;
   if (!ok) return fail(PFN_ERR_UNSUPPORTED, "head dim %d unsupported (32/64/128/256)", dh);
   if (d->emsize > 2048) return fail(PFN_ERR_UNSUPPORTED, "emsize > 2048 unsupported by the LayerNorm kernels");
-  if (d->schedule & ~(PFN_SCHED_TOP_LAYER_ALL_ROWS | PFN_SCHED_FUSE_LN_WIDE | PFN_SCHED_SEPARATE_LNBWD | PFN_SCHED_DETERMINISTIC | PFN_SCHED_NO_KEY_CENTERING | PFN_SCHED_FUSE_Q_PROJECTION | PFN_SCHED_KEY_CENTERING | PFN_SCHED_F32_RESIDUAL)) return fail(PFN_ERR_ARGUMENT, "unknown schedule bits 0x%x", d->schedule);
+  if (d->schedule & ~(PFN_SCHED_TOP_LAYER_ALL_ROWS | PFN_SCHED_FUSE_LN_WIDE | PFN_SCHED_SEPARATE_LNBWD | PFN_SCHED_DETERMINISTIC | PFN_SCHED_NO_KEY_CENTERING | PFN_SCHED_FUSE_Q_PROJECTION | PFN_SCHED_KEY_CENTERING | PFN_SCHED_F32_RESIDUAL | PFN_SCHED_KEEP_DSRC)) return fail(PFN_ERR_ARGUMENT, "unknown schedule bits 0x%x", d->schedule);
   if (!(d->dropout >= 0.f && d->dropout < 1.f)) return fail(PFN_ERR_ARGUMENT, "dropout %g outside [0, 1)", (double)d->dropout);
   return PFN_OK;
 }
@@ -118,6 +118,9 @@
 struct Ws {
   float* x0; char* x0_t;
   char* xaug_t;
+  int xaug_pitch;
+  float *emb_g1, *emb_g2, *emb_cs1, *emb_cs2, *emb_acc;
+  int64_t emb_g_bytes;
   float* embacc;
   float* xaug_amax;
   std::vector<LayerWs> layer;
@@ -150,6 +153,12 @@
   return d.precision == PFN_PREC_FP16 && !(d.schedule & PFN_SCHED_F32_RESIDUAL) && d.nlayers > 0 && d.dropout == 0.f && d.emsize >= 1024 && d.emsize % 8 == 0 && !ln_fusable;
 }
 
+static int xaug_row_pitch(const pfn_model_desc& d) {
+  const int aug = emb_aug_width(d.num_features);
+  if (aug == 0) return 32;
+  return (prec_is16(d.precision) && d.nlayers > 0 && d.emsize % 256 == 0 && d.dropout == 0.f) ? 256 : aug;
+}
+
 Ws carve(const pfn_model_desc& d, int B, int S, char* base) {
   Ws w;
   const int64_t M = (int64_t)B * S, E = d.emsize, F = d.nhid, es = esize(d.precision);
@@ -158,8 +167,15 @@
   auto take = [&](int64_t nbytes) { char* p = base ? base + cur : nullptr; cur = align_up(cur + nbytes, 256); return p; };
   w.x0 = (float*)take(M * E * 4); w.x0_t = take(M * E * es);
   const int64_t aug = emb_aug_width(d.num_features) > 0 ? emb_aug_width(d.num_features) : 32;
-  w.xaug_t = take(M * aug * es); w.embacc = (float*)take(E * aug * 4);
+  w.xaug_pitch = xaug_row_pitch(d);
+  w.xaug_t = take(M * w.xaug_pitch * es); w.embacc = (float*)take(E * aug * 4);
   w.xaug_amax = (float*)take(aug * 4);
+  w.emb_g1 = w.emb_g2 = w.emb_cs1 = w.emb_cs2 = w.emb_acc = nullptr; w.emb_g_bytes = 0;
+  if (w.xaug_pitch == 256) {
+    w.emb_g_bytes = (4 * E * 256 + 4 * E + E * aug) * 4;
+    w.emb_g1 = (float*)take(w.emb_g_bytes);
+    if (w.emb_g1) { w.emb_g2 = w.emb_g1 + 3 * E * 256; w.emb_cs1 = w.emb_g2 + E * 256; w.emb_cs2 = w.emb_cs1 + 3 * E; w.emb_acc = w.emb_cs2 + E; }
+  }
   w.layer.resize(d.nlayers);
   for (auto& l : w.layer) {
     l.qkv = take(M * 3 * E * es); l.ctx = take(M * E * es); l.lse = (float*)take((int64_t)B * d.nhead * S * 4);
@@ -316,6 +332,9 @@
 bool emb_gemm(const pfn_model_desc& d, bool custom_encoder) {
   return !custom_encoder && prec_is16(d.precision) && d.nlayers > 0 && emb_aug_width(d.num_features) > 0 && d.emsize % 8 == 0;
 }
+bool emb_from_wgrad(const pfn_model_desc& d, const Ws& w, bool custom_encoder, float pdrop) {
+  return emb_gemm(d, custom_encoder) && w.emb_g1 != nullptr && pdrop == 0.f && !(d.schedule & (PFN_SCHED_DETERMINISTIC | PFN_SCHED_KEEP_DSRC));
+}
 bool predict_dsrc_is_t(const pfn_model_desc& d) { return d.nlayers > 0 && prec_is16(d.precision); }
 
 struct Resid { const float* plain; const void* y; const float* mean; const float* rstd; const float* gamma; const float* beta; };
@@ -409,7 +428,7 @@
   auto one_by_one = [&](size_t i0, size_t n) {
     for (size_t i = i0; i < i0 + n; ++i) {
       const TnProblem& t = probs[i];
-      GemmTN g = tn(t.A, t.lda, t.B, t.ldb, t.C, t.ldc, rows, t.Pv ? t.Pv : t.P, t.Q, t.colsum);
+      GemmTN g = tn(t.A, t.lda, t.B, t.ldb, t.C, t.ldc, t.M ? t.M : rows, t.Pv ? t.Pv : t.P, t.Q, t.colsum);
       if (det) g.max_splits = 1;
       g.scale_amax = lsc;
       PFN_TRY(launch_gemm_tn(g, prec, s));
@@ -671,7 +690,7 @@
     e.x = x; e.x_st = x_st; e.x_sb = x_sb; e.y = y; e.y_st = y_st; e.y_sb = y_sb;
     e.wx = params + L.enc_w; e.bx = params + L.enc_b; e.wy = params + L.yenc_w; e.by = params + L.yenc_b;
     e.out_f32 = w.x0; e.out_t = w.x0_t; e.S = S; e.B = B; e.nf = d->num_features; e.E = E; e.sep = sep; e.sep_of = sep_of;
-    e.xaug_ld = emb_aug_width(d->num_features);
+    e.xaug_ld = emb_aug_width(d->num_features); e.xaug_pitch = w.xaug_pitch;
     e.xaug_t = e.xaug_ld > 0 ? w.xaug_t : nullptr;
     e.xaug_amax = nullptr;
     if (e.xaug_t && prec == PFN_PREC_FP16) {
@@ -1079,11 +1098,14 @@
   };
   const bool emb_t = emb_gemm(*d, dsrc_sbe != nullptr);
   const bool fuse_lnb = d->nlayers > 0 && lnbwd_fusable(m, pl, lsc, view(0, false), M);
+  const bool emb_wg = emb_from_wgrad(*d, w, dsrc_sbe != nullptr, pdrop);
+  if (emb_wg && hipMemsetAsync(w.emb_g1, 0, w.emb_g_bytes, s) != hipSuccess) return fail(PFN_ERR_LAUNCH, "hipMemsetAsync(emb_g)");
   auto launch_weight_gradients = [&](int l_hi, int l_lo) -> int {
     std::vector<TnProblem> probs, probs_top;
     auto add = [&](const void* A, long lda, const void* Bm, long ldb, float* C, long ldc, int P, int Q, float* colsum, bool compact = false) {
       TnProblem t; memset(&t, 0, sizeof(t)); t.A = A; t.lda = lda; t.B = Bm; t.ldb = ldb; t.C = C; t.ldc = ldc; t.P = P; t.Q = Q; t.colsum = colsum;
-      (compact ? probs_top : probs).push_back(t);
+      if (compact) { t.M = Mt; if (Mt > 0) probs_top.push_back(t); }
+      else probs.push_back(t);
     };
     for (int l = l_hi; l >= l_lo; --l) {
       const LayerP& p = L.layer[l];
@@ -1096,7 +1118,11 @@
       add(drop ? a.dy1m_t : (top ? w.top_dy1_t : a.dy1_t), E, top ? w.top_ctx_t : a.ctx, E, grads + p.w_o, E, E, E, (drop || fuse_lnb) ? grads + p.b_o : nullptr, top);
       add(a.dqkv_t, 3 * E, xin_t, E, grads + p.w_in, E, 3 * E, E, grads + p.b_in);
     }
-    PFN_TRY(launch_tn_set(probs_top, Mt, prec, det, lsc, PFN_PROF_WGRAD + 1, s));
+    if (emb_wg && l_lo == 0) {
+      add(w.layer[0].dqkv_t, 3 * E, w.xaug_t, w.xaug_pitch, w.emb_g1, 256, 3 * E, 256, w.emb_cs1);
+      add(w.layer[0].dy1_t, E, w.xaug_t, w.xaug_pitch, w.emb_g2, 256, E, 256, w.emb_cs2);
+    }
+    probs.insert(probs.end(), probs_top.begin(), probs_top.end());
     PFN_TRY(launch_tn_set(probs, M, prec, det, lsc, PFN_PROF_WGRAD, s));
     return PFN_OK;
   };
@@ -1149,7 +1175,7 @@
       PFN_TRY(launch_attn_bwd(at, prec, s));
     }
     const LayerGrads below = l > 0 ? view(l - 1, false) : LayerGrads{};
-    PFN_TRY(layer_backward_dx(m, t, a.dqkv_t, a.dy1_t, M, pl, lsc, fuse_lnb && l > 0 ? &below : nullptr, w.gA, w.gA_t, l == 0 && !emb_t, 0));
+    if (!(l == 0 && emb_wg)) PFN_TRY(layer_backward_dx(m, t, a.dqkv_t, a.dy1_t, M, pl, lsc, fuse_lnb && l > 0 ? &below : nullptr, w.gA, w.gA_t, l == 0 && !emb_t, 0));
     if (l == split_at) {
       PFN_TRY(launch_weight_gradients(d->nlayers - 1, split_at));
       on_first_group(user);
@@ -1159,9 +1185,12 @@
   const int aug = emb_aug_width(d->num_features);
   if (dsrc_sbe) {
     PFN_TRY(launch_bse_to_sbe(w.gA, dsrc_sbe, S, B, E, s, lsc));
+  } else if (emb_wg) {
+    PFN_TRY(launch_embed_grad_finish(params + L.layer[0].w_in, w.emb_g1, w.emb_g2, w.emb_cs1, w.emb_cs2, 256, w.emb_acc, grads + L.enc_b, E, aug, s));
+    PFN_TRY(launch_embed_grad_scatter(w.emb_acc, grads + L.enc_w, grads + L.yenc_w, grads + L.yenc_b, E, d->num_features, prec == PFN_PREC_FP16 ? w.xaug_amax : nullptr, s));
   } else if (emb_t) {
     if (hipMemsetAsync(w.embacc, 0, sizeof(float) * E * aug, s) != hipSuccess) return fail(PFN_ERR_LAUNCH, "memset");
-    GemmTN g = tn(w.gA_t, E, w.xaug_t, aug, w.embacc, aug, M, E, aug, grads + L.enc_b);
+    GemmTN g = tn(w.gA_t, E, w.xaug_t, w.xaug_pitch, w.embacc, aug, M, E, aug, grads + L.enc_b);
     g.scale_amax = lsc;
     g.max_splits = det ? 1 : 128;
     PFN_TRY(launch_gemm_tn(g, prec, s));
@@ -1187,6 +1216,8 @@
   const Layout L = make_layout(*d);
   hipStream_t s = (hipStream_t)stream;
   const bool emb_t = emb_gemm(*d, false);
+  if (emb_from_wgrad(*d, w, false, 0.f))
+    return fail(PFN_ERR_ARGUMENT, "pfn_stack_input_grads: this descriptor's backward does not keep d(src); set PFN_SCHED_KEEP_DSRC in the descriptor of the backward and of this call");
   EmbedInGradArgs e; memset(&e, 0, sizeof(e));
   e.dsrc = emb_t ? (const void*)w.gA_t : (const void*)w.gA; e.dsrc_prec = emb_t ? prec : PFN_PREC_F32;
   e.wx = params + L.enc_w; e.wy = params + L.yenc_w;
@@ -1534,6 +1565,28 @@
   PFN_TRY(launch_gemm_tn_group(g, prec, (hipStream_t)stream));
   return PFN_OK;
 }
+int pfn_op_gemm_tn_group_rows(int n, const void* const* A, const int64_t* lda, const void* const* B, const int64_t* ldb, float* const* C,
+                              const int64_t* ldc, const int32_t* P, const int32_t* Q, float* const* colsum, const int32_t* M, int splits, int prec, void* stream) {
+  if (n < 1 || n > TN_GROUP_MAX || !A || !lda || !B || !ldb || !C || !ldc || !P || !Q || !M) return fail(PFN_ERR_ARGUMENT, "bad gemm_tn_group_rows arguments");
+  GemmTNGroup g;
+  memset(&g, 0, sizeof(g));
+  g.n = n; g.splits = splits;
+  for (int i = 0; i < n; ++i) {
+    if (M[i] < 0) return fail(PFN_ERR_ARGUMENT, "gemm_tn_group_rows: problem %d has %d rows", i, M[i]);
+    TnProblem& t = g.p[i];
+    t.A = A[i]; t.lda = lda[i]; t.B = B[i]; t.ldb = ldb[i]; t.C = C[i]; t.ldc = ldc[i]; t.P = P[i]; t.Q = Q[i];
+    t.colsum = colsum ? colsum[i] : nullptr;
+    t.M = M[i] > 0 ? M[i] : -1;
+  }
+  PFN_TRY(launch_gemm_tn_group(g, prec, (hipStream_t)stream));
+  return PFN_OK;
+}
+int pfn_op_gemm_tn_group_plan(int n, const int32_t* P, const int32_t* Q, const int32_t* M, int splits, int cus, int32_t* chunks, int32_t* chunk_rows) {
+  if (n < 1 || n > TN_GROUP_MAX || !P || !Q || !M || !chunks || !chunk_rows || splits < 0) { fail(PFN_ERR_ARGUMENT, "bad gemm_tn_group_plan arguments"); return -1; }
+  for (int i = 0; i < n; ++i)
+    if (P[i] <= 0 || Q[i] <= 0 || P[i] % 256 || Q[i] % 256) { fail(PFN_ERR_UNSUPPORTED, "gemm_tn_group_plan: P and Q must be multiples of 256"); return -1; }
+  return tn_group_plan(n, P, Q, M, splits, cus, chunks, chunk_rows);
+}
 int pfn_op_gemm_ln(const void* A, int64_t lda, const void* B, int64_t ldb, int M, int N, int K, const float* bias,
                    const float* resid, const float* ry, const float* rmean, const float* rrstd, const float* rgamma, const float* rbeta,
                    const float* gamma, const float* beta, float eps, float* y, float* mean, float* rstd, void* x_t, int prec, void* stream) {
diff --git a/transformerscandobayesianinference_amd/csrc/pfn_kernels.h b/transformerscandobayesianinference_amd/csrc/pfn_kernels.h
--- a/transformerscandobayesianinference_amd/csrc/pfn_kernels.h
+++ b/transformerscandobayesianinference_amd/csrc/pfn_kernels.h
@@ -112,11 +112,13 @@
   long lda, ldb, ldc;
   int P, Q;
   int Pv;
+  int M;
 };
 struct GemmTNGroup {
   TnProblem p[TN_GROUP_MAX];
-  int tile_start[TN_GROUP_MAX + 1];
-  int n, M, splits, m_chunk;
+  int item_start[TN_GROUP_MAX + 1];
+  int chunk[TN_GROUP_MAX];
+  int n, M, splits;
   int debug_mask;
   const float* scale_amax;
 };
@@ -153,6 +155,7 @@
 int launch_gemm_lnbwd(const GemmLNB& g, int precision, hipStream_t stream);
 
 bool gemm_tn_group_supported(const TnProblem& p);
+int tn_group_plan(int n, const int* P, const int* Q, const int* M, int splits, int cus, int* chunks, int* chunk_rows);
 int launch_gemm_tn_group(GemmTNGroup g, int precision, hipStream_t stream);
 
 struct AttnArgs {
@@ -233,6 +236,7 @@
   float* out_f32; void* out_t;
   void* xaug_t;
   int xaug_ld;
+  int xaug_pitch;
   const float* xaug_amax;
   int S, B, nf, E, sep;
   const int* sep_of;
@@ -258,6 +262,7 @@
 };
 int launch_embed_bwd(const EmbedBwdArgs& a, hipStream_t s);
 int launch_embed_grad_scatter(const float* acc, float* dwx, float* dwy, float* dby, int E, int nf, const float* xaug_amax, hipStream_t s);
+int launch_embed_grad_finish(const float* w_in, const float* g1, const float* g2, const float* cs1, const float* cs2, int ldg, float* acc, float* dbx, int E, int aug, hipStream_t s);
 struct EmbedInGradArgs {
   const void* dsrc; int dsrc_prec;
   const float* wx; const float* wy;
diff --git a/transformerscandobayesianinference_amd/csrc/rowwise.hip b/transformerscandobayesianinference_amd/csrc/rowwise.hip
--- a/transformerscandobayesianinference_amd/csrc/rowwise.hip
+++ b/transformerscandobayesianinference_amd/csrc/rowwise.hip
@@ -235,7 +235,7 @@
   const long ntok = (long)a.B * a.S;
   const long t0 = (long)blockIdx.x * EMB_TOK;
   const int nfp = a.nf + 2;
-  if (a.xaug_t && threadIdx.x < a.xaug_ld) xexp[threadIdx.x] = xaug_col_exp(a.xaug_amax, threadIdx.x);
+  if (a.xaug_t && threadIdx.x < min(a.xaug_ld, 128)) xexp[threadIdx.x] = xaug_col_exp(a.xaug_amax, threadIdx.x);
   for (int i = threadIdx.x; i < EMB_TOK * nfp; i += 256) {
     const int tk = i / nfp, f = i % nfp;
     const long tok = t0 + tk;
@@ -253,7 +253,7 @@
   T* out_t = reinterpret_cast<T*>(a.out_t);
   if (a.xaug_t) {
     T* xa = reinterpret_cast<T*>(a.xaug_t);
-    const int aug = a.xaug_ld;
+    const int aug = a.xaug_pitch;
     for (int i = threadIdx.x; i < EMB_TOK * aug; i += 256) {
       const int tk = i / aug, f = i % aug;
       if (t0 + tk < ntok) xa[(t0 + tk) * aug + f] = (T)(f < nfp ? ldexpf(xs[tk * nfp + f], -xexp[f]) : 0.f);
@@ -441,6 +441,58 @@
   hipLaunchKernelGGL(embed_grad_scatter_kernel, dim3((E * (nf + 2) + 255) / 256), dim3(256), 0, s, acc, dwx, dwy, dby, E, nf, xaug_amax);
   return PFN_LAUNCH_OK();
 }
+constexpr int EGF_SLICES = 8, EGF_F = 8, EGF_E = 64, EGF_J = 4;
+__global__ __launch_bounds__(EGF_E * EGF_J) void embed_grad_finish_kernel(const float* __restrict__ w_in, const float* __restrict__ g1, const float* __restrict__ g2,
+                                                                          const float* __restrict__ cs1, const float* __restrict__ cs2, int ldg,
+                                                                          float* acc, float* dbx, int E, int aug) {
+  __shared__ float red[EGF_J][EGF_F][EGF_E];
+  const int te = threadIdx.x % EGF_E, tj = threadIdx.x / EGF_E;
+  const int e = blockIdx.x * EGF_E + te;
+  const bool live = e < E;
+  const int ec = live ? e : E - 1;
+  const int rows = 3 * E, per = (rows + EGF_SLICES * EGF_J - 1) / (EGF_SLICES * EGF_J);
+  const int j0 = (blockIdx.z * EGF_J + tj) * per, j1 = min(rows, j0 + per);
+  const int f0 = blockIdx.y * EGF_F;
+  const bool bias = f0 >= aug;
+  float v[EGF_F];
+#pragma unroll
+  for (int k = 0; k < EGF_F; ++k) v[k] = 0.f;
+  if (bias) {
+#pragma unroll 8
+    for (int j = j0; j < j1; ++j) v[0] += w_in[(long)j * E + ec] * cs1[j];
+  } else {
+#pragma unroll 8
+    for (int j = j0; j < j1; ++j) {
+      const float w = w_in[(long)j * E + ec];
+      const float* g = g1 + (long)j * ldg + f0;
+#pragma unroll
+      for (int k = 0; k < EGF_F; ++k) v[k] += w * g[k];
+    }
+  }
+#pragma unroll
+  for (int k = 0; k < EGF_F; ++k) red[tj][k][te] = v[k];
+  __syncthreads();
+  if (tj != 0 || !live) return;
+#pragma unroll
+  for (int k = 0; k < (bias ? 1 : EGF_F); ++k) {
+    float t = 0.f;
+#pragma unroll
+    for (int q = 0; q < EGF_J; ++q) t += red[q][k][te];
+    if (bias) {
+      if (blockIdx.z == 0) t += cs2[e];
+      unsafeAtomicAdd(dbx + e, t);
+    } else {
+      if (blockIdx.z == 0) t += g2[(long)e * ldg + f0 + k];
+      unsafeAtomicAdd(acc + (long)e * aug + f0 + k, t);
+    }
+  }
+}
+int launch_embed_grad_finish(const float* w_in, const float* g1, const float* g2, const float* cs1, const float* cs2, int ldg, float* acc, float* dbx, int E, int aug,
+                             hipStream_t s) {
+  if (aug <= 0 || aug > ldg || aug % EGF_F) return PFN_ERR_UNSUPPORTED;
+  hipLaunchKernelGGL(embed_grad_finish_kernel, dim3((E + EGF_E - 1) / EGF_E, aug / EGF_F + 1, EGF_SLICES), dim3(EGF_E * EGF_J), 0, s, w_in, g1, g2, cs1, cs2, ldg, acc, dbx, E, aug);
+  return PFN_LAUNCH_OK();
+}
 __global__ __launch_bounds__(256) void embed_input_grad_kernel(EmbedInGradArgs a, int R, int fc) {
   extern __shared__ float eig_sm[];
   float* ds = eig_sm;
diff --git a/transformerscandobayesianinference_amd/hipops.py b/transformerscandobayesianinference_amd/hipops.py
--- a/transformerscandobayesianinference_amd/hipops.py
+++ b/transformerscandobayesianinference_amd/hipops.py
@@ -42,6 +42,30 @@
     P = I(*[p[0].shape[1] for p in problems]); Q = I(*[p[1].shape[1] for p in problems])
     cs = VP(*[(p[3].data_ptr() if p[3] is not None else None) for p in problems])
     _hip.check(_hip.lib().pfn_op_gemm_tn_group(n, A, lda, B, ldb, C, ldc, P, Q, cs, M, splits, PREC_OF[problems[0][0].dtype], sp()), 'pfn_op_gemm_tn_group')
+
+
+def gemm_tn_group_rows(problems, splits=0):
+    import ctypes
+    n = len(problems)
+    VP, L, I = ctypes.c_void_p * n, ctypes.c_int64 * n, ctypes.c_int32 * n
+    A = VP(*[p[0].data_ptr() for p in problems]); lda = L(*[p[0].stride(0) for p in problems])
+    B = VP(*[p[1].data_ptr() for p in problems]); ldb = L(*[p[1].stride(0) for p in problems])
+    C = VP(*[p[2].data_ptr() for p in problems]); ldc = L(*[p[2].stride(0) for p in problems])
+    P = I(*[p[0].shape[1] for p in problems]); Q = I(*[p[1].shape[1] for p in problems])
+    M = I(*[p[0].shape[0] for p in problems])
+    assert all(p[0].shape[0] == p[1].shape[0] for p in problems)
+    cs = VP(*[(p[3].data_ptr() if p[3] is not None else None) for p in problems])
+    _hip.check(_hip.lib().pfn_op_gemm_tn_group_rows(n, A, lda, B, ldb, C, ldc, P, Q, cs, M, splits, PREC_OF[problems[0][0].dtype], sp()), 'pfn_op_gemm_tn_group_rows')
+
+
+def gemm_tn_group_plan(shapes, splits=0, cus=256):
+    import ctypes
+    n = len(shapes)
+    I = ctypes.c_int32 * n
+    P, Q, M = I(*[s[0] for s in shapes]), I(*[s[1] for s in shapes]), I(*[s[2] for s in shapes])
+    chunks, rows = I(), I()
+    items = _hip.check(_hip.lib().pfn_op_gemm_tn_group_plan(n, P, Q, M, splits, cus, chunks, rows), 'pfn_op_gemm_tn_group_plan')
+    return items, list(chunks), list(rows)
 
 
 SUMS_16BIT = 256
diff --git a/transformerscandobayesianinference_amd/transformer.py b/transformerscandobayesianinference_amd/transformer.py
--- a/transformerscandobayesianinference_amd/transformer.py
+++ b/transformerscandobayesianinference_amd/transformer.py
@@ -108,6 +108,9 @@
         if desc is not model._desc:
             raise RuntimeError('backward through an inference-precision forward: the forward of this graph ran the eval_precision kernels')
         model._attach_grads()
+        if src is None and (ctx.needs_input_grad[2] or ctx.needs_input_grad[3]):
+            desc = _hip.ModelDesc(*desc.key())
+            desc.schedule |= _hip.SCHED_KEEP_DSRC
         dlogits = dlogits.contiguous().float()
         dsrc = None
         if src is not None:
```
